# JuliaQuantumControl/GRAPE.jl

Hardware: AMD Instinct MI355X
Metric: GRAPE gradient evals/sec (N=64, 1000 steps, 128 traj) (higher is better)
Workload: dtype f64

## Files before the change

### grape.jl_amd/api.py

```python
from __future__ import annotations

import ctypes as C
import os
import subprocess
import sys

import numpy as np

_HERE = os.path.dirname(os.path.abspath(__file__))
_CSRC = os.path.join(_HERE, "csrc")
_LIBNAME = "libgrape_hip.so"

J_T_SM, J_T_SS, J_T_RE = 0, 1, 2
GRAD_GRADGEN, GRAD_TAYLOR = 0, 1
PROP_EXP, PROP_SERIES = 0, 1
ABI_VERSION = 7

STATUS = {0: "GRAPE_OK", -1: "GRAPE_ERR_INVALID", -2: "GRAPE_ERR_HIP", -3: "GRAPE_ERR_CHI_NORM",
          -4: "GRAPE_ERR_SINGULAR", -5: "GRAPE_ERR_TAYLOR", -6: "GRAPE_ERR_NO_CONTROLS", -7: "GRAPE_ERR_AGAIN",
          -8: "GRAPE_ERR_HOST"}

EXPORTS = ["grape_create", "grape_destroy", "grape_eval", "grape_forward", "grape_backward",
           "grape_forward_device", "grape_backward_device", "grape_check", "grape_get_propagator",
           "grape_get_tau_grads", "grape_get_storage", "grape_get_timings", "grape_reset_timings", "grape_get_work", "grape_get_cert_table",
           "grape_last_error", "grape_abi_version", "grape_set_fused_sweeps", "grape_get_sums", "grape_backward_xi",
           "grape_get_final_states", "grape_backward_chi",
           "grape_get_time_gradient", "grape_set_tlist", "grape_eval_batch", "grape_get_batch_info", "grape_create_open",
           "grape_hvp", "grape_get_hvp_info", "grape_open_time_gradient", "grape_open_hvp", "grape_get_open_hvp_info",
           "grape_open_eval_batch", "grape_get_open_batch_info", "grape_open_set_running_cost", "grape_open_backward_xi",
           "grape_hvp_forward", "grape_hvp_backward", "grape_hvp_backward_chi",
           "grape_open_hvp_forward", "grape_open_hvp_backward", "grape_open_hvp_backward_chi"]


class GrapeHipError(RuntimeError):
    def __init__(self, code, msg):
        super().__init__(f"{STATUS.get(code, code)}: {msg}")
        self.code = code


class _Problem(C.Structure):
    _fields_ = [("abi_version", C.c_int32), ("N", C.c_int32), ("L", C.c_int32), ("K", C.c_int32),
                ("K_total", C.c_int32), ("N_T", C.c_int32), ("functional", C.c_int32),
                ("gradient_method", C.c_int32), ("hc_per_traj", C.c_int32), ("device", C.c_int32),
                ("tlist", C.c_void_p), ("H0", C.c_void_p), ("Hc", C.c_void_p), ("shape", C.c_void_p),
                ("psi0", C.c_void_p), ("target", C.c_void_p), ("weights", C.c_void_p),
                ("chi_min_norm", C.c_double), ("taylor_max_order", C.c_int32),
                ("taylor_tolerance", C.c_double),
                ("Dpen", C.c_void_p), ("dpen_per_traj", C.c_int32), ("lambda_b", C.c_double),
                ("prop_method", C.c_int32), ("prop_tolerance", C.c_double),
                ("ndev", C.c_int32), ("devices", C.c_void_p), ("taylor_no_check", C.c_int32)]


class _Lindblad(C.Structure):
    _fields_ = [("J", C.c_int32), ("cops_per_traj", C.c_int32), ("cops", C.c_void_p)]


def library_path() -> str:
    return os.path.join(_CSRC, _LIBNAME)


def build_asm(verbose: bool = False, workdir: str | None = None) -> str:
    asm_dir = os.path.join(_CSRC, "asm")
    work = workdir or asm_dir
    kernels = (("gen_t16.py", "expm_t16_asm"), ("gen_t16p.py", "expm_t16p_asm"), ("gen_t16p.py", "expm_t16p4_asm"), ("gen_t18g.py", "expm_t18g_asm"), ("gen_t18gp.py", "expm_t18gp_asm"), ("gen_d3.py", "deriv3_asm"), ("gen_d3s.py", "deriv3s_asm"), ("gen_d3s.py", "deriv3g_asm"),
               ("gen_lg.py", "lg_gemm_asm"), ("gen_d4.py", "deriv4_asm_128"), ("gen_d4.py", "deriv4_asm_256"))
    co_path, emb_s, emb_o = os.path.join(work, "grape_asm.co"), os.path.join(work, "asm_embed.S"), os.path.join(work, "asm_embed.o")
    llvm = "/opt/rocm/lib/llvm/bin"
    cmds, objs = [], []
    for gen_py, name in kernels:
        s_path, o_path = os.path.join(work, name + ".s"), os.path.join(work, name + ".o")
        gen = subprocess.run([sys.executable, os.path.join(asm_dir, gen_py), s_path], capture_output=True, text=True)
        if verbose or gen.returncode:
            print(gen.stdout, gen.stderr)
        if gen.returncode:
            raise RuntimeError(gen_py + " failed")
        cmds.append([os.path.join(llvm, "clang"), "-x", "assembler", "-target", "amdgcn-amd-amdhsa", "-mcpu=gfx950", "-c", s_path, "-o", o_path])
        objs.append(o_path)
    cmds.append([os.path.join(llvm, "ld.lld"), "-shared"] + objs + ["-o", co_path])
    with open(emb_s, "w") as f:
        f.write('\t.section .rodata\n\t.globl grape_asm_co_start\n\t.globl grape_asm_co_end\n\t.p2align 12\n'
                'grape_asm_co_start:\n\t.incbin "grape_asm.co"\ngrape_asm_co_end:\n\t.byte 0\n'
                '\t.section .note.GNU-stack,"",@progbits\n')
    cmds.append(["gcc", "-c", "-fPIC", "asm_embed.S", "-o", "asm_embed.o"])
    for c in cmds:
        res = subprocess.run(c, capture_output=True, text=True, cwd=work)
        if verbose or res.returncode:
            print(" ".join(c), res.stdout, res.stderr)
        if res.returncode:
            raise RuntimeError("assembling the gfx950 kernels failed")
    return emb_o


def _sources():
    srcs = [os.path.join(_CSRC, f) for f in ("grape_hip.hip", "grape_t18.hip", "grape_kernels.hip.h", "grape_large.hip.h",
                                             "grape_series.hip.h", "grape_cheby.hip.h", "grape_t18.hip.h", "grape_t18_coeffs.h",
                                             "grape_deriv3.hip.h", "grape_timegrad.hip.h", "grape_batch.hip.h", "grape_lindblad.hip.h", "grape_lindblad_tg.hip.h", "grape_hvp.hip.h", "grape_hvp_split.hip.h", "grape_lindblad_hvp.hip.h", "grape_lindblad_hvp_split.hip.h", "grape_lindblad_batch.hip.h", "grape_lindblad_rc.hip.h", "grape_devmem.h", "grape_cert.hip.h", os.path.join("asm", "gen_t16.py"), os.path.join("asm", "gen_t16p.py"), os.path.join("asm", "gen_t18g.py"), os.path.join("asm", "gen_t18gp.py"), os.path.join("asm", "gen_d3.py"), os.path.join("asm", "gen_d3s.py"), os.path.join("asm", "gen_lg.py"), os.path.join("asm", "gen_d4.py"), os.path.join("asm", "gcn.py"))]
    return srcs, os.path.join(_HERE, "..", "include", "grape_hip.h")


def _up_to_date(out: str) -> bool:
    srcs, hdr = _sources()
    return os.path.exists(out) and all(os.path.getmtime(out) >= os.path.getmtime(s) for s in srcs + [hdr])


def build_library(force: bool = False, verbose: bool = False, extra_flags=(), out: str | None = None) -> str:
    import fcntl
    import shutil
    import tempfile
    out = out or library_path()
    if not force and _up_to_date(out):
        return out
    srcs, _ = _sources()
    with open(os.path.join(_CSRC, ".build.lock"), "w") as lockf:
        fcntl.flock(lockf, fcntl.LOCK_EX)
        if not force and _up_to_date(out):
            return out
        work = tempfile.mkdtemp(prefix="_build_", dir=_CSRC)
        procs = []
        try:
            base = ["hipcc", "--offload-arch=gfx950", "-O3", "-std=c++17", "-fPIC", "-Wno-unused-value"] + list(extra_flags)
            objs = [os.path.join(work, "grape_hip.o"), os.path.join(work, "grape_t18.o")]
            cmds = [base + ["-cuid=grapehip0", "-c", srcs[0], "-o", objs[0]],
                    base + ["-cuid=grapehip1", "-mllvm", "-amdgpu-mfma-vgpr-form", "-c", srcs[1], "-o", objs[1]]]
            procs = [subprocess.Popen(c, stdout=subprocess.PIPE, stderr=subprocess.STDOUT, text=True) for c in cmds]
            objs.append(build_asm(verbose, workdir=work))
            outs = [p.communicate()[0] for p in procs]
            if verbose or any(p.returncode for p in procs):
                print("\n".join(outs))
            if any(p.returncode for p in procs):
                raise RuntimeError("hipcc failed building " + out)
            tmp_so = os.path.join(work, _LIBNAME)
            res = subprocess.run(["hipcc", "--offload-arch=gfx950", "-shared", "-fPIC"] + objs + ["-o", tmp_so], capture_output=True, text=True)
            if verbose or res.returncode:
                print(res.stdout, res.stderr)
            if res.returncode:
                raise RuntimeError("hipcc failed linking " + out)
            asm_dir = os.path.join(_CSRC, "asm")
            for f in os.listdir(work):
                if f.endswith(".s") or f.endswith(".co"):
                    os.replace(os.path.join(work, f), os.path.join(asm_dir, f))
            os.replace(tmp_so, out)
        finally:
            for p in procs:
                if p.poll() is None:
                    p.kill()
                    p.communicate()
            shutil.rmtree(work, ignore_errors=True)
    return out


_lib = None


def load_library():
    global _lib
    if _lib is not None:
        return _lib
    path = library_path()
    if not os.path.exists(path):
        raise GrapeHipError(-2, f"{path} not built; run __graft_entry__.build() (no CPU fallback exists)")
    try:
        import torch
    except ImportError:
        pass
    lib = C.CDLL(path)
    vp, dp, ip = C.c_void_p, C.POINTER(C.c_double), C.c_int
    lib.grape_create.argtypes = [C.POINTER(vp), C.POINTER(_Problem)]
    lib.grape_create_open.argtypes = [C.POINTER(vp), C.POINTER(_Problem), C.POINTER(_Lindblad)]
    lib.grape_destroy.argtypes = [vp]
    lib.grape_destroy.restype = None
    lib.grape_eval.argtypes = [vp, vp, dp, vp, vp, vp]
    lib.grape_forward.argtypes = [vp, vp, vp]
    lib.grape_backward.argtypes = [vp, vp, vp]
    lib.grape_forward_device.argtypes = [vp, vp, vp, vp]
    lib.grape_backward_device.argtypes = [vp, vp, vp, vp]
    lib.grape_check.argtypes = [vp, vp]
    lib.grape_get_propagator.argtypes = [vp, ip, ip, vp]
    lib.grape_get_tau_grads.argtypes = [vp, vp]
    lib.grape_get_storage.argtypes = [vp, ip, vp]
    lib.grape_get_timings.argtypes = [vp, vp, ip]
    lib.grape_get_work.argtypes = [vp, vp, ip]
    lib.grape_get_cert_table.argtypes = [vp, vp, vp, vp]
    lib.grape_reset_timings.argtypes = [vp]
    lib.grape_set_fused_sweeps.argtypes = [vp, ip]
    lib.grape_get_sums.argtypes = [vp, vp]
    lib.grape_get_final_states.argtypes = [vp, vp]
    lib.grape_backward_chi.argtypes = [vp, vp, vp]
    lib.grape_backward_xi.argtypes = [vp, vp, vp, vp, C.c_double, vp]
    lib.grape_get_time_gradient.argtypes = [vp, vp]
    lib.grape_open_time_gradient.argtypes = [vp, vp]
    lib.grape_set_tlist.argtypes = [vp, vp]
    lib.grape_eval_batch.argtypes = [vp, ip, vp, vp, vp, vp]
    lib.grape_get_batch_info.argtypes = [vp, vp, ip]
    lib.grape_hvp.argtypes = [vp, ip, vp, vp]
    lib.grape_get_hvp_info.argtypes = [vp, vp, ip]
    lib.grape_hvp_forward.argtypes = [vp, ip, vp, vp, vp, vp]
    lib.grape_hvp_backward.argtypes = [vp, ip, vp, vp, vp]
    lib.grape_hvp_backward_chi.argtypes = [vp, ip, vp, vp, vp]
    lib.grape_open_hvp.argtypes = [vp, ip, vp, vp]
    lib.grape_get_open_hvp_info.argtypes = [vp, vp, ip]
    lib.grape_open_hvp_forward.argtypes = [vp, ip, vp, vp, vp, vp]
    lib.grape_open_hvp_backward.argtypes = [vp, ip, vp, vp, vp]
    lib.grape_open_hvp_backward_chi.argtypes = [vp, ip, vp, vp, vp]
    lib.grape_open_eval_batch.argtypes = [vp, ip, vp, vp, vp, vp]
    lib.grape_get_open_batch_info.argtypes = [vp, vp, ip]
    lib.grape_open_set_running_cost.argtypes = [vp, vp, ip, C.c_double]
    lib.grape_open_backward_xi.argtypes = [vp, vp, vp, vp, C.c_double, vp]
    lib.grape_last_error.argtypes = [vp]
    lib.grape_last_error.restype = C.c_char_p
    lib.grape_abi_version.restype = ip
    _lib = lib
    return lib


def _c128(a, shape=None):
    a = np.ascontiguousarray(a, dtype=np.complex128)
    if shape is not None:
        assert a.shape == tuple(shape), (a.shape, shape)
    return a


class GrapeHip:

    def __init__(self, H0, Hc, tlist, psi0, target, weights=None, functional=J_T_SM,
                 gradient_method=GRAD_GRADGEN, shape=None, K_total=None, device=0,
                 chi_min_norm=0.0, taylor_max_order=0, taylor_tolerance=0.0, D=None, lambda_b=0.0,
                 prop_method=PROP_EXP, prop_tolerance=0.0, devices=None, taylor_check_convergence=True):
        self._lib = load_library()
        H0 = np.asarray(H0)
        if H0.ndim != 3 or H0.shape[1] != H0.shape[2]:
            raise ValueError(f"H0 must be [K, N, N], got {H0.shape}")
        K, N = H0.shape[0], H0.shape[1]
        Hc = np.asarray(Hc)
        per_traj = Hc.ndim == 4
        if Hc.ndim not in (3, 4) or Hc.shape[-2:] != (N, N) or (per_traj and Hc.shape[0] != K):
            raise ValueError(f"Hc must be [L, N, N] or [K, L, N, N] with N = {N}, K = {K}, got {Hc.shape}")
        L = Hc.shape[1] if per_traj else Hc.shape[0]
        tlist = np.ascontiguousarray(tlist, dtype=np.float64)
        if tlist.ndim != 1 or len(tlist) < 2:
            raise ValueError("tlist must hold at least two time points")
        N_T = len(tlist) - 1
        if weights is not None and np.shape(weights) != (K,):
            raise ValueError(f"weights must be [K] = [{K}], got {np.shape(weights)}")
        if D is not None and np.shape(D) not in ((N, N), (K, N, N)):
            raise ValueError(f"D must be [N, N] or [K, N, N] with N = {N}, K = {K}, got {np.shape(D)}")
        self.N, self.L, self.K, self.N_T = N, L, K, N_T
        self.K_total = K if K_total is None else int(K_total)
        self.functional = functional
        self._H0 = _c128(np.swapaxes(H0, -1, -2), (K, N, N))
        self._Hc = _c128(np.swapaxes(Hc, -1, -2))
        self._psi0 = _c128(psi0, (K, N))
        self._target = None if target is None else _c128(target, (K, N))
        self._tlist = tlist
        self._weights = None if weights is None else np.ascontiguousarray(weights, dtype=np.float64)
        self._shape = None if shape is None else np.ascontiguousarray(shape, dtype=np.float64).reshape(L, N_T)
        p = _Problem()
        p.abi_version = ABI_VERSION
        p.N, p.L, p.K, p.K_total, p.N_T = N, L, K, self.K_total, N_T
        p.functional, p.gradient_method, p.hc_per_traj, p.device = functional, gradient_method, int(per_traj), device
        p.tlist = self._tlist.ctypes.data
        p.H0 = self._H0.ctypes.data
        p.Hc = self._Hc.ctypes.data
        p.shape = None if self._shape is None else self._shape.ctypes.data
        p.psi0 = self._psi0.ctypes.data
        p.target = None if self._target is None else self._target.ctypes.data
# ... 147 lines not shown

    def hvp_forward(self, V, final_states=False):
        v, nv = self._hvp_dirs(V)
        dtau = np.empty((nv, self.K), dtype=np.complex128)
        dsums = np.empty(nv, dtype=np.complex128)
        dpsi = np.empty((nv, self.K, self.N), dtype=np.complex128) if final_states else None
        self._chk(self._lib.grape_hvp_forward(self._h, nv, v.ctypes.data, dtau.ctypes.data, dsums.ctypes.data,
                                              dpsi.ctypes.data if final_states else None))
        if v.ndim == 1:
            dtau, dsums, dpsi = dtau[0], dsums[0], (dpsi[0] if final_states else None)
        return (dtau, dsums, dpsi) if final_states else (dtau, dsums)

    def hvp_backward(self, f_total, df_total):
        one = np.ndim(df_total) == 0
        df = np.ascontiguousarray(df_total, dtype=np.complex128)
        if np.ndim(df_total) > 1 or df.size == 0:
            raise ValueError(f"df_total must be a complex scalar or [nv] with nv >= 1, got {np.shape(df_total)}")
        nv = df.size
        out = np.empty((nv, self.L * self.N_T))
        f = np.array([complex(f_total).real, complex(f_total).imag], dtype=np.float64)
        self._chk(self._lib.grape_hvp_backward(self._h, nv, f.ctypes.data, df.ctypes.data, out.ctypes.data))
        return out[0] if one else out

    def hvp_backward_chi(self, chi, dchi):
        chi = np.ascontiguousarray(chi, dtype=np.complex128)
        d = np.ascontiguousarray(dchi, dtype=np.complex128)
        if chi.shape != (self.K, self.N):
            raise ValueError(f"chi must be [K, N] = [{self.K}, {self.N}], got {chi.shape}")
        if d.ndim not in (2, 3) or d.shape[-2:] != (self.K, self.N) or d.size == 0:
            raise ValueError(f"dchi must be [K, N] = [{self.K}, {self.N}] or [nv, {self.K}, {self.N}] with nv >= 1, got {d.shape}")
        nv = 1 if d.ndim == 2 else d.shape[0]
        out = np.empty((nv, self.L * self.N_T))
        self._chk(self._lib.grape_hvp_backward_chi(self._h, nv, chi.ctypes.data, d.ctypes.data, out.ctypes.data))
        return out[0] if d.ndim == 2 else out

    def set_tlist(self, tlist):
        t = np.ascontiguousarray(tlist, dtype=np.float64)
        if t.shape != (self.N_T + 1,):
            raise ValueError(f"tlist must have N_T + 1 = {self.N_T + 1} points, got {t.shape}")
        self._chk(self._lib.grape_set_tlist(self._h, t.ctypes.data))
        self._tlist = t

    def forward_device(self, d_pulsevals_ptr, d_out_ptr, stream=0):
        self._chk(self._lib.grape_forward_device(self._h, d_pulsevals_ptr, d_out_ptr, stream))

    def backward_device(self, d_f_ptr, d_G_ptr, stream=0):
        self._chk(self._lib.grape_backward_device(self._h, d_f_ptr, d_G_ptr, stream))

    def set_fused_sweeps(self, on=True):
        return bool(self._lib.grape_set_fused_sweeps(self._h, int(bool(on))))

    def check(self, stream=0):
        self._chk(self._lib.grape_check(self._h, stream))

    def propagator(self, k, n):
        out = np.empty((self.N, self.N), dtype=np.complex128)
        self._chk(self._lib.grape_get_propagator(self._h, k, n, out.ctypes.data))
        return out.T.copy()

    def tau_grads(self):
        out = np.empty((self.K, self.L, self.N_T), dtype=np.complex128)
        self._chk(self._lib.grape_get_tau_grads(self._h, out.ctypes.data))
        return out

    def storage(self, which=0):
        out = np.empty((self.K, self.N_T + 1, self.N), dtype=np.complex128)
        self._chk(self._lib.grape_get_storage(self._h, which, out.ctypes.data))
        return out

    def timings(self):
        ms = np.full(8, -1.0)
        self._lib.grape_get_timings(self._h, ms.ctypes.data, 8)
        out = dict(zip(["expm", "forward", "backward", "deriv", "reduce", "total"], ms[:6].tolist()))
        if ms[6] >= 0.0:
            out["host_enqueue"] = float(ms[6])
        if ms[7] >= 0.0:
            out["gradient_allreduce_us"] = float(ms[7]) * 1e3
        return out

    def reset_timings(self):
        self._chk(self._lib.grape_reset_timings(self._h))

    def work(self):
        w = np.zeros(20)
        self._lib.grape_get_work(self._h, w.ctypes.data, 20)
        return dict(cells=w[0], squarings=w[1], flop_expm=w[2], flop_deriv=w[3], deriv_orders=w[4],
                    pivoted_cells=w[5], expm_cells=w[6], series_terms=w[7], series_steps=w[8],
                    t18_mfma_flop=w[9], t18_squarings=w[10], t18_cells=w[11], matrix_free_fallback=w[12], t16_cells=w[13],
                    asm_kernel=w[14], asm_deriv_kernel=w[15], asm_blocked_products=w[16],
                    walk_steps=w[17], scan_block=w[18], t16_certified=w[19])

    def cert_table(self):
        dims = np.zeros(3, np.int32)
        self._chk(self._lib.grape_get_cert_table(self._h, dims.ctypes.data, None, None))
        KC, n8, n6 = (int(x) for x in dims)
        coef, exps = np.zeros((KC, n8 + n6)), np.zeros(n8 + n6, np.int32)
        if n8 + n6:
            self._chk(self._lib.grape_get_cert_table(self._h, dims.ctypes.data, coef.ctypes.data, exps.ctypes.data))
        ex = np.stack([(exps >> (4 * l)) & 15 for l in range(self.L)], axis=1) if n8 + n6 else np.zeros((0, self.L), np.int32)
        return coef[:, :n8], coef[:, n8:], ex


def liouvillian(H, cops=()):
    H = np.asarray(H, dtype=np.complex128)
    d = H.shape[0]
    if H.shape != (d, d):
        raise ValueError(f"H must be [d, d], got {H.shape}")
    eye = np.eye(d)
    heff = H.copy()
    for A in cops:
        A = np.asarray(A, dtype=np.complex128)
        heff = heff - 0.5j * (A.conj().T @ A)
    out = np.kron(eye, heff) - np.kron(heff.conj(), eye)
    for A in cops:
        A = np.asarray(A, dtype=np.complex128)
        out = out + 1j * np.kron(A.conj(), A)
    return out


class GrapeHipOpen(GrapeHip):

    def __init__(self, H0, Hc, cops, tlist, rho0, target, weights=None, functional=J_T_SM, shape=None, K_total=None,
                 device=0, chi_min_norm=0.0, prop_tolerance=0.0):
        self._lib = load_library()
        H0 = np.asarray(H0)
        if H0.ndim != 3 or H0.shape[1] != H0.shape[2]:
            raise ValueError(f"H0 must be [K, d, d], got {H0.shape}")
        K, N = H0.shape[0], H0.shape[1]
        Hc = np.asarray(Hc)
        per_traj = Hc.ndim == 4
        if Hc.ndim not in (3, 4) or Hc.shape[-2:] != (N, N) or (per_traj and Hc.shape[0] != K):
            raise ValueError(f"Hc must be [L, d, d] or [K, L, d, d] with d = {N}, K = {K}, got {Hc.shape}")
        L = Hc.shape[1] if per_traj else Hc.shape[0]
        tlist = np.ascontiguousarray(tlist, dtype=np.float64)
        if tlist.ndim != 1 or len(tlist) < 2:
            raise ValueError("tlist must hold at least two time points")
        N_T = len(tlist) - 1
        if weights is not None and np.shape(weights) != (K,):
            raise ValueError(f"weights must be [K] = [{K}], got {np.shape(weights)}")
        cops = None if cops is None or np.size(cops) == 0 else np.asarray(cops)
        cops_per_traj = cops is not None and cops.ndim == 4
        if cops is not None and (cops.ndim not in (3, 4) or cops.shape[-2:] != (N, N) or (cops_per_traj and cops.shape[0] != K)):
            raise ValueError(f"cops must be [J, d, d] or [K, J, d, d] with d = {N}, K = {K}, got {cops.shape}")
        self.N, self.L, self.K, self.N_T = N, L, K, N_T
        self.J = 0 if cops is None else cops.shape[-3]
        self.K_total = K if K_total is None else int(K_total)
        self.functional = functional
        self.prop_method = PROP_EXP
        self.lambda_b = 0.0
        self._H0 = _c128(np.swapaxes(H0, -1, -2), (K, N, N))
        self._Hc = _c128(np.swapaxes(Hc, -1, -2))
        self._cops = None if cops is None else _c128(np.swapaxes(cops, -1, -2))
        self._psi0 = _c128(np.swapaxes(np.asarray(rho0), -1, -2), (K, N, N))
        self._target = None if target is None else _c128(np.swapaxes(np.asarray(target), -1, -2), (K, N, N))
        self._tlist = tlist
        self._weights = None if weights is None else np.ascontiguousarray(weights, dtype=np.float64)
        self._shape = None if shape is None else np.ascontiguousarray(shape, dtype=np.float64).reshape(L, N_T)
        p = _Problem()
        p.abi_version = ABI_VERSION
        p.N, p.L, p.K, p.K_total, p.N_T = N, L, K, self.K_total, N_T
        p.functional, p.gradient_method, p.hc_per_traj, p.device = functional, GRAD_GRADGEN, int(per_traj), device
        p.tlist = self._tlist.ctypes.data
        p.H0 = self._H0.ctypes.data
        p.Hc = self._Hc.ctypes.data
        p.shape = None if self._shape is None else self._shape.ctypes.data
        p.psi0 = self._psi0.ctypes.data
        p.target = None if self._target is None else self._target.ctypes.data
        p.weights = None if self._weights is None else self._weights.ctypes.data
        p.chi_min_norm = chi_min_norm
        p.prop_method, p.prop_tolerance = PROP_EXP, float(prop_tolerance)
        d = _Lindblad()
        d.J, d.cops_per_traj = self.J, int(cops_per_traj)
        d.cops = None if self._cops is None else self._cops.ctypes.data
        self._h = C.c_void_p()
        rc = self._lib.grape_create_open(C.byref(self._h), C.byref(p), C.byref(d))
        if rc:
            msg = self._lib.grape_last_error(None).decode()
            self._h = None
            raise GrapeHipError(rc, msg)

    def eval(self, pulsevals, gradient=True, want_psiT=False):
        x = np.ascontiguousarray(pulsevals, dtype=np.float64)
        assert x.size == self.L * self.N_T
# ... 143 lines not shown
```

### grape.jl_amd/csrc/asm/gen_d3.py

```python
import os
import struct
import sys

sys.path.insert(0, os.path.dirname(os.path.abspath(__file__)))
from gcn import Prog, V, A, S, VCC, EXEC, Neg, kernel_text

NT = 4
NP = 64
LDT = 17
TILE_B = 16 * LDT * 8
NTILE = NT * (NT + 1) // 2
MAT_B = NTILE * 2 * TILE_B
KERNARG = 160
VPLANE_B = NP * 16 * 16
ECON_MIN = 16
PAIRS_OFF = 32768
ECON_OFF = 32768
ECON_TAB_B = 512


def tile_index(ti, tj):
    assert ti <= tj
    return ti * NT - ti * (ti - 1) // 2 + (tj - ti)


def dbits(x):
    b = struct.unpack("<Q", struct.pack("<d", x))[0]
    return b & 0xFFFFFFFF, b >> 32


class GenD3:
    def __init__(self, name="deriv3_asm", LMAX=2, opts=None):
        assert 1 <= LMAX <= 2
        self.p = Prog(name)
        self.p.soft_vm_flush = True
        self.LMAX = LMAX
        self.opts = dict(opts or {})
        self.lds_bytes = (1 + LMAX) * MAT_B
        self.s_H0, self.s_Hc, self.s_eps, self.s_shape, self.s_dts = S(4, 2), S(6, 2), S(8, 2), S(10, 2), S(12, 2)
        self.s_fw, self.s_bw, self.s_rho = S(14, 2), S(16, 2), S(18, 2)
        self.s_tg, self.s_park, self.s_flags, self.s_stats = S(20, 2), S(22, 2), S(24, 2), S(26, 2)
        self.s_bflag, self.s_inv = S(28, 2), S(30, 2)
        self.s_K, self.s_L, self.s_NT, self.s_hcpt, self.s_wpt, self.s_bpk, self.s_mcap, self.s_maxm = (S(32 + i) for i in range(8))
        self.s_tol2, self.s_deep, self.s_nblk = S(40, 2), S(42), S(43)
        self.s_wave, self.s_slot, self.s_k, self.s_part, self.s_bq, self.s_n0 = (S(44 + i) for i in range(6))
        self.s_m, self.s_M, self.s_conv, self.s_kl = S(50), S(51), S(52), S(53)
        self.s_valid = S(54, 2)
        self.s_fwb, self.s_bwb, self.s_pw = S(56, 2), S(58, 2), S(60, 2)
        self.s_a, self.s_b = S(62, 2), S(64, 2)
        self.s_invm = S(66, 2)
        self.s_t = [S(68 + i) for i in range(8)]
        self.s_pb = [S(76 + 2 * t, 2) for t in range(4)]
        self.s_save = S(84, 2)
        self.s_rhov = S(86, 2)
        self.s_lo16 = S(88, 2)
        self.s_capb, self.s_econ = S(90), S(91)
        self.s_sig = S(92, 2)
        self.v_tid, self.v_lane = V(0), V(1)
        self.v_BD = [V(2 + 2 * op) for op in range(3)]
        self.v_BM = [V(3 + 2 * op) for op in range(3)]
        self.v_fwoff, self.v_bwoff, self.v_poff, self.v_tgoff, self.v_nc8, self.v_zero = V(8), V(9), V(10), V(11), V(12), V(13)
        self.v_dt = V(14, 2)
        self.v_e = [V(16, 2), V(18, 2)]
        self.v_sfac, self.v_nn = V(20, 2), V(22, 2)
        self.v_dr = [V(24, 2), V(28, 2)]
        self.v_di = [V(26, 2), V(30, 2)]
        self.f_re = [V(32 + 2 * rt, 2) for rt in range(4)]
        self.f_im = [V(40 + 2 * rt, 2) for rt in range(4)]
        self.f_as = [V(48 + 2 * rt, 2) for rt in range(4)]
        self.P = [[V(56 + 8 * (4 * j + rt), 8) for rt in range(4)] for j in range(3)]
        self.SUM = [[V(152 + 8 * (4 * j + rt), 8) for rt in range(4)] for j in range(2)]
        self.TMP = [V(216 + 8 * i, 8) for i in range(5)]
        self.VEC = [[A(8 * (4 * j + t), 8) for t in range(4)] for j in range(3)]
        self.CHI = [[A(96 + 8 * (4 * j + t), 8) for t in range(4)] for j in range(2)]
        self.ULAND = A(160, 64)
        self.SHK = [A(224, 2), A(226, 2)]

    def smov64(self, dst, x):
        lo, hi = dbits(x)
        self.p.salu("s_mov_b32", dst.sub(0), lo)
        self.p.salu("s_mov_b32", dst.sub(1), hi)

    def udiv(self, q, r, num, den, tag):
        p = self.p
        i, t = self.s_t[6], self.s_t[7]
        p.salu("s_mov_b32", q, 0)
        p.salu("s_mov_b32", r, 0)
        p.salu("s_mov_b32", i, 31)
        p.label(f"L_div_{tag}")
        p.salu("s_lshl_b32", r, r, 1)
        p.salu("s_lshr_b32", t, num, i)
        p.salu("s_and_b32", t, t, 1)
        p.salu("s_or_b32", r, r, t)
        p.s_cmp("s_cmp_ge_u32", r, den)
        p.s_branch("s_cbranch_scc0", f"L_div_skip_{tag}")
        p.salu("s_sub_u32", r, r, den)
        p.salu("s_lshl_b32", t, 1, i)
        p.salu("s_or_b32", q, q, t)
# ... 581 lines not shown
```

### grape.jl_amd/csrc/grape_cert.hip.h

```cpp
#pragma once

#include <hip/hip_runtime.h>

#include <cstdint>
#include <map>
#include <vector>

#define GRAPE_CERT_LMAX 4

struct CertMonomials {
    std::vector<uint32_t> key;
    std::map<uint32_t, int> index;
    CertMonomials(int M, int d) {
        gen(M, d, 0, 0u);
        for (size_t i = 0; i < key.size(); ++i) index[key[i]] = (int)i;
    }
    int size() const { return (int)key.size(); }

private:
    void gen(int M, int left, int a, uint32_t k) {
        if (a == M - 1) { key.push_back(k | ((uint32_t)left << (4 * a))); return; }
        for (int e = left; e >= 0; --e) gen(M, left - e, a + 1, k | ((uint32_t)e << (4 * a)));
    }
};

struct CertJobs {
    std::vector<int> row, pair;
    void from(const std::vector<std::vector<int>> &lists) {
        row.assign(1, 0);
        pair.clear();
        for (const auto &l : lists) {
            pair.insert(pair.end(), l.begin(), l.end());
            row.push_back((int)pair.size() / 2);
        }
    }
};

struct CertPlan {
    int M, n2, n3, n4, n6, n8, nmat;
    CertJobs mm2, mm34, tr;
    std::vector<int> exps;
    explicit CertPlan(int L) {
        M = L + 1;
        const CertMonomials m2(M, 2), m3(M, 3), m4(M, 4), m6(M, 6), m8(M, 8);
        n2 = m2.size(); n3 = m3.size(); n4 = m4.size(); n6 = m6.size(); n8 = m8.size();
        const int o2 = M, o3 = o2 + n2, o4 = o3 + n3;
        nmat = o4 + n4;
        auto var = [&](int a) { return (uint32_t)1 << (4 * a); };
        std::vector<std::vector<int>> l2(n2), l34(n3 + n4), lt(n8 + n6);
        for (int a = 0; a < M; ++a)
            for (int b = 0; b < M; ++b) { auto &l = l2[m2.index.at(var(a) + var(b))]; l.push_back(a); l.push_back(b); }
        for (int i = 0; i < n2; ++i)
            for (int c = 0; c < M; ++c) { auto &l = l34[m3.index.at(m2.key[i] + var(c))]; l.push_back(o2 + i); l.push_back(c); }
        for (int i = 0; i < n2; ++i)
            for (int j = 0; j < n2; ++j) { auto &l = l34[n3 + m4.index.at(m2.key[i] + m2.key[j])]; l.push_back(o2 + i); l.push_back(o2 + j); }
        for (int i = 0; i < n4; ++i)
            for (int j = 0; j < n4; ++j) { auto &l = lt[m8.index.at(m4.key[i] + m4.key[j])]; l.push_back(o4 + i); l.push_back(o4 + j); }
        for (int i = 0; i < n3; ++i)
            for (int j = 0; j < n3; ++j) { auto &l = lt[n8 + m6.index.at(m3.key[i] + m3.key[j])]; l.push_back(o3 + i); l.push_back(o3 + j); }
        mm2.from(l2); mm34.from(l34); tr.from(lt);
        for (int i = 0; i < n8; ++i) exps.push_back((int)(m8.key[i] >> 4));
        for (int i = 0; i < n6; ++i) exps.push_back((int)(m6.key[i] >> 4));
    }
};

__global__ void __launch_bounds__(256) cert_load_kernel(const double *H0f, const double *Hcf, const int *rep, int kc0, int hc_per_traj, int L,
                                                        int N, int NP, int nmat, double2 *scratch) {
    const int a = blockIdx.x, c = blockIdx.y, kc = kc0 + c, k = rep ? rep[kc] : kc;
    const size_t pp = (size_t)NP * NP;
    const double *src = a == 0 ? H0f + (size_t)k * 2 * pp : Hcf + ((size_t)(hc_per_traj ? k : 0) * L + (a - 1)) * 2 * pp;
    double2 *dst = scratch + ((size_t)c * nmat + a) * N * N;
    for (int e = threadIdx.x; e < N * N; e += 256) {
        const int i = e / N, j = e - i * N;
        dst[e] = make_double2(src[(size_t)i * NP + j], src[pp + (size_t)i * NP + j]);
    }
}

__global__ void __launch_bounds__(256) cert_mm_kernel(double2 *scratch, int nmat, int N, int dst0, const int *row, const int *pair) {
    double2 *base = scratch + (size_t)blockIdx.y * nmat * N * N;
    double2 *dst = base + (size_t)(dst0 + blockIdx.x) * N * N;
    const int p0 = row[blockIdx.x], p1 = row[blockIdx.x + 1];
    for (int e = threadIdx.x; e < N * N; e += 256) {
        const int i = e / N, j = e - i * N;
        double sr = 0., si = 0.;
        for (int q = p0; q < p1; ++q) {
            const double2 *A = base + (size_t)pair[2 * q] * N * N + (size_t)i * N, *B = base + (size_t)pair[2 * q + 1] * N * N + j;
            double tr = 0., ti = 0.;
            for (int k = 0; k < N; ++k) {
                const double2 x = A[k], y = B[(size_t)k * N];
                tr += x.x * y.x - x.y * y.y;
                ti += x.x * y.y + x.y * y.x;
            }
            sr += tr; si += ti;
        }
        dst[e] = make_double2(sr, si);
    }
}

__global__ void __launch_bounds__(256) cert_trace_kernel(const double2 *scratch, int nmat, int N, const int *row, const int *pair, int nt,
                                                         double *table) {
    __shared__ double red[256];
    const double2 *base = scratch + (size_t)blockIdx.y * nmat * N * N;
    const int p0 = row[blockIdx.x], p1 = row[blockIdx.x + 1];
    double sum = 0.;
    for (int q = p0; q < p1; ++q) {
        const double2 *A = base + (size_t)pair[2 * q] * N * N, *B = base + (size_t)pair[2 * q + 1] * N * N;
        double t = 0.;
        for (int e = threadIdx.x; e < N * N; e += 256) {
            const int i = e / N, j = e - i * N;
            const double2 x = A[e], y = B[(size_t)j * N + i];
            t += x.x * y.x - x.y * y.y;
        }
        sum += t;
    }
    red[threadIdx.x] = sum;
    __syncthreads();
    for (int off = 128; off >= 1; off >>= 1) {
        if ((int)threadIdx.x < off) red[threadIdx.x] += red[threadIdx.x + off];
        __syncthreads();
    }
    if (threadIdx.x == 0) table[(size_t)blockIdx.y * nt + blockIdx.x] = red[0];
}
```

### grape.jl_amd/csrc/grape_deriv3.hip.h

```cpp
#pragma once
#include "grape_t18.hip.h"

struct Deriv3Args {
    Deriv2Args d;
    const double *H0f, *Hcf;
    int wpt;
    int skip_if_flagged;
};

template <int NT>
struct D3Lds {
    static constexpr int LDT = 17, TILE = 16 * LDT;
    static constexpr int NTILE = NT * (NT + 1) / 2, MAT = NTILE * 2 * TILE;
    static constexpr int tile(int ti, int tj) { return ti * NT - ti * (ti - 1) / 2 + (tj - ti); }
};

template <int NT>
struct D3Vec {
    d4 re[NT], im[NT];
};
template <int NT>
__device__ __forceinline__ void d3_finish(D3Vec<NT> &) {}
#define MFMA64_NEGA(a, b, c) __builtin_amdgcn_mfma_f64_16x16x4f64((a), (b), (c), 0, 0, 1)

// ... 90 lines not shown
#pragma unroll
                    for (int tj = 0; tj < NT; ++tj) {
                        const bool full = H0G && m == 0;
                        if (tj < ti && !full) continue;
                        const size_t o = (size_t)(16 * ti + row) * NP + 16 * tj + col;
                        const int q_ = full ? ti * NT + tj : LY::tile(ti, tj);
                        double *dst = d3sm + (m == 0 ? (size_t)0 : (size_t)H0SZ + (size_t)(m - 1) * LY::MAT) + (size_t)q_ * 2 * LY::TILE
                                      + row * LY::LDT + col;
                        dst[0] = src[o];
                        dst[LY::TILE] = src[pp + o];
                    }
            }
            __syncthreads();
            k_loaded = k;
        }
        for (int bq = part * 4 + wave; bq < a.batches_per_k; bq += 4 * g.wpt) {
            const int batch = k * a.batches_per_k + bq;
            const int n0 = bq * 16, n = n0 + c;
            const bool valid = n < a.N_T;
            const int nc = valid ? n : a.N_T - 1;
            const double dt = a.dts[nc];
            double e[LMAX], sh[LMAX];
#pragma unroll
            for (int l = 0; l < LMAX; ++l) {
                sh[l] = (l < L && a.shape) ? a.shape[(size_t)l * a.N_T + nc] : 1.0;
                e[l] = l < L ? a.eps[(size_t)l * a.N_T + nc] * sh[l] : 0.;
            }
            auto apply = [&](const D3Vec<NT> &v, Strip<NT> &sum, auto each, auto adj) __attribute__((always_inline)) {
                if constexpr (!H0G) d3_product<NT, D3_HERM>(sum, d3sm, v, lane);
                else if constexpr (decltype(adj)::value) d3_product<NT, D3_FULL_ADJ>(sum, d3sm, v, lane);
                else d3_product<NT, D3_FULL>(sum, d3sm, v, lane);
#pragma unroll
                for (int l = 0; l < LMAX; ++l) {
                    if (l < L) {
                        Strip<NT> q;
                        d3_product<NT, D3_HERM>(q, d3sm + (size_t)H0SZ + (size_t)l * LY::MAT, v, lane);
                        each(l, q);
#pragma unroll
                        for (int t = 0; t < NT; ++t) { sum.re[t] += e[l] * q.re[t]; sum.im[t] += e[l] * q.im[t]; }
                    }
                }
            };
            D3Vec<NT> v;
#pragma unroll
            for (int t = 0; t < NT; ++t)
#pragma unroll
                for (int r = 0; r < 4; ++r) {
                    const int row = 16 * t + 4 * r + rg;
                    const double2 p = a.fw[((size_t)k * (a.N_T + 1) + nc) * NP + row];
                    v.re[t][r] = valid ? p.x : 0.; v.im[t][r] = valid ? p.y : 0.;
                    const size_t o = (size_t)row * 16 + c;
                    park[o] = v.re[t][r]; park[vplane + o] = v.im[t][r];
                }
            d3_finish<NT>(v);
            int M = 0, converged = 0;
            const int deg = (a.batch_econ && a.batch_flag && a.econ_pairs) ? a.batch_flag[a.nbatch_total + batch] : 0;
            const int capb = (deg && deg - 1 <= mcap) ? deg - 1 : mcap;
            const double *pairs = nullptr;
            for (int m = 1; m <= capb; ++m) {
                Strip<NT> sum;
                apply(v, sum, [](int, const Strip<NT> &) {}, std::false_type());
                const double sfac = dt / (double)m;
                double nn = 0.;
#pragma unroll
                for (int t = 0; t < NT; ++t)
#pragma unroll
                    for (int r = 0; r < 4; ++r) {
                        const double ur = sfac * sum.im[t][r], ui = -sfac * sum.re[t][r];
                        v.re[t][r] = ur; v.im[t][r] = ui;
                        if (m < a.maxm) {
                            const size_t o = (size_t)m * 2 * vplane + (size_t)(16 * t + 4 * r + rg) * 16 + c;
                            park[o] = ur; park[vplane + o] = ui;
                        }
                        nn += ur * ur + ui * ui;
                    }
                d3_finish<NT>(v);
                nn += __shfl_xor(nn, 16, 64);
                nn += __shfl_xor(nn, 32, 64);
                M = m;
                if (m >= 2 && __all(nn < a.tol * a.tol)) { converged = 1; break; }
            }
            if (!converged && capb != mcap) {
                M = deg; converged = 1;
                pairs = a.econ_pairs + (size_t)(deg - 16) * 64;
            }
            Strip<NT> chi;
#pragma unroll
            for (int t = 0; t < NT; ++t)
#pragma unroll
                for (int r = 0; r < 4; ++r) {
                    const int row = 16 * t + 4 * r + rg;
                    const double2 x = a.bw[((size_t)k * (a.N_T + 1) + nc + 1) * NP + row];
                    chi.re[t][r] = valid ? x.x : 0.; chi.im[t][r] = valid ? x.y : 0.;
                    v.re[t][r] = chi.re[t][r]; v.im[t][r] = chi.im[t][r];
                }
            d3_finish<NT>(v);
            double dr[LMAX], di[LMAX];
#pragma unroll
            for (int l = 0; l < LMAX; ++l) { dr[l] = 0.; di[l] = 0.; }
            for (int aa = M - 1; aa >= 0; --aa) {
                const double inv = pairs ? pairs[2 * aa] : 1.0 / (double)(aa + 1), sfac = dt * (pairs ? pairs[2 * aa + 1] : inv);
                Strip<NT> u;
#pragma unroll
                for (int t = 0; t < NT; ++t)
#pragma unroll
                    for (int r = 0; r < 4; ++r) {
                        const size_t o = (size_t)aa * 2 * vplane + (size_t)(16 * t + 4 * r + rg) * 16 + c;
                        u.re[t][r] = park[o]; u.im[t][r] = park[vplane + o];
                    }
                Strip<NT> sum;
                apply(v, sum, [&](int l, const Strip<NT> &q) {
                    double sr = 0., si = 0.;
#pragma unroll
                    for (int t = 0; t < NT; ++t)
#pragma unroll
                        for (int r = 0; r < 4; ++r) {
                            sr += q.re[t][r] * u.re[t][r] + q.im[t][r] * u.im[t][r];
                            si += q.re[t][r] * u.im[t][r] - q.im[t][r] * u.re[t][r];
                        }
#pragma unroll
                    for (int ll = 0; ll < LMAX; ++ll)
                        if (ll == l) { dr[ll] += inv * sr; di[ll] += inv * si; }
                }, std::true_type());
                if (aa > 0) {
#pragma unroll
                    for (int t = 0; t < NT; ++t) {
                        v.re[t] = chi.re[t] - sfac * sum.im[t];
                        v.im[t] = chi.im[t] + sfac * sum.re[t];
                    }
                    d3_finish<NT>(v);
                }
            }
            const double rho = a.rho[k];
#pragma unroll
            for (int l = 0; l < LMAX; ++l) {
                if (l < L) {
                    double Dr = dr[l], Di = di[l];
                    Dr += __shfl_xor(Dr, 16, 64); Di += __shfl_xor(Di, 16, 64);
                    Dr += __shfl_xor(Dr, 32, 64); Di += __shfl_xor(Di, 32, 64);
                    if (lane < 16 && valid) {
                        const double f = rho * dt * sh[l];
                        a.tg[((size_t)k * L + l) * a.N_T + n] = make_double2(f * Di, -f * Dr);
                    }
                }
            }
            if (lane == 0) {
                const bool redone = a.batch_flag && a.batch_flag[batch];
                if (!converged && !redone) {
                    if (a.deep_redo && a.max_order > mcap) atomicAdd(&a.flags[7], 1);
                    else atomicOr(&a.flags[0], 4);
                }
                if (!redone) stat_add(a.stats, 8, (unsigned long long)M * (unsigned long long)min(16, a.N_T - n0));
            }
        }
    }
}
```

### grape.jl_amd/csrc/grape_econ_coeffs.h

```cpp
#pragma once
#define ECON_NSETS 4
#define ECON_MAXDEG 21
static const int ECON_DEG[4] = {16, 17, 19, 21};
static const double ECON_THETAS[4] = {1.36, 1.6, 2.0, 2.72};
static const double ECON_TABS[4][21][2] = {
    {
        {0.99999999999999980529, 0.0},
        {0.49999999999999995125, 0.5000000000000000486},
        {0.33333333333332434652, 0.33333333333332437902},
        {0.24999999999999620304, 0.25000000000000294314},
        {0.19999999999926497087, 0.19999999999926800844},
        {0.16666666666628327988, 0.16666666666689580415},
        {0.14285714278897023749, 0.14285714278929885474},
        {0.12499999995893169073, 0.12500000001858273294},
        {0.11111110479818800082, 0.11111110483469316255},
        {0.099999995732971707361, 0.10000000141460258699},
        {0.09090855395893132458, 0.090908557838025207959},
        {0.083332932906864668469, 0.083333425111719705549},
        {0.076884663733727549698, 0.07688503317535548076},
        {0.071397325340398044236, 0.071432996940482527776},
        {0.064640984384933717337, 0.064669273650506011373},
        {0.06071810592472735844, 0.062620855279837302966},
    },
    {
        {0.99999999999999999455, 0.0},
        {0.4999999999999993495, 0.49999999999999935223},
        {0.33333333333333310332, 0.33333333333333353698},
        {0.24999999999996339023, 0.24999999999996356274},
        {0.19999999999998274025, 0.20000000000001202807},
        {0.16666666666399540022, 0.16666666666400978334},
        {0.14285714285565865098, 0.14285714285794830793},
        {0.12499999979320799999, 0.12499999979450668039},
        {0.11111111098113255448, 0.11111111116494766568},
        {0.099999984471020328113, 0.099999984588001011055},
        {0.090909080095443414331, 0.090909094212698174517},
        {0.08333227990005947407, 0.083332289812445550663},
        {0.076922274865354993361, 0.07692324726745345143},
        {0.071369128617731144553, 0.071369872773579570035},
        {0.066617645519177640728, 0.066673130855455625664},
        {0.060046505756126821541, 0.060090691475870164317},
        {0.056647927484758038627, 0.058962556159000548588},
    },
    {
        {0.99999999999999999921, 0.0},
        {0.49999999999999992552, 0.49999999999999992591},
        {0.33333333333333330714, 0.33333333333333335679},
        {0.24999999999999664644, 0.24999999999999666609},
        {0.19999999999999844313, 0.20000000000000112597},
        {0.16666666666646977996, 0.16666666666647107735},
        {0.14285714285703602551, 0.14285714285720478555},
        {0.12499999998758439536, 0.12499999998767787304},
        {0.11111111110354300887, 0.11111111111457910189},
        {0.099999999224287985445, 0.099999999231099277407},
        {0.090909090388332223524, 0.090909091093524965459},
        {0.08333328800342905667, 0.083333288480790928176},
        {0.076923043819425117041, 0.076923085662418433957},
        {0.071426233987298557027, 0.071426264725411121612},
        {0.066664825888945511032, 0.066667007511954072934},
        {0.062401392779846247146, 0.062403115833826611183},
        {0.058740346168331276547, 0.058833168170990150001},
        {0.052549019651987751242, 0.052623435248405465345},
        {0.04992966106659680109, 0.052786333172829262077},
    },
    {
        {0.99999999999999999857, 0.0},
        {0.49999999999999991112, 0.49999999999999991184},
        {0.33333333333333330218, 0.33333333333333336144},
        {0.24999999999999735495, 0.24999999999999737832},
        {0.19999999999999878645, 0.20000000000000090249},
        {0.16666666666656360018, 0.16666666666656461147},
        {0.14285714285708797303, 0.14285714285717631573},
        {0.12499999999564817792, 0.12499999999569620152},
        {0.11111111110852316905, 0.11111111111239145534},
        {0.099999999815243407927, 0.099999999817572555781},
        {0.090909090788705288148, 0.090909090956665826485},
        {0.083333325825673231936, 0.083333325936026708004},
        {0.076923071625269883499, 0.076923078555417816465},
        {0.071428292264000648122, 0.071428297183374011482},
        {0.066666455064462201818, 0.066666715618252914584},
        {0.06249097939752106286, 0.062491177746585624593},
        {0.058816230400073814299, 0.058824720550794186756},
        {0.055319711558037046927, 0.055326576656644222471},
        {0.052428888318170015129, 0.052652407896601588093},
        {0.04557403849702946584, 0.045750228205306646811},
        {0.043596611933927011585, 0.047830533974697739686},
    },
};
```

### grape.jl_amd/csrc/grape_hip.hip

```cpp
#include "../../include/grape_hip.h"
#include "grape_kernels.hip.h"
#include "grape_t18_coeffs.h"
#include "grape_econ_coeffs.h"
#include "grape_large.hip.h"
#include "grape_series.hip.h"
#include "grape_cheby.hip.h"
#include "grape_timegrad.hip.h"
#include "grape_lindblad.hip.h"
#include "grape_lindblad_tg.hip.h"
#include "grape_hvp.hip.h"
#include "grape_hvp_split.hip.h"
#include "grape_lindblad_hvp.hip.h"
#include "grape_lindblad_hvp_split.hip.h"
#include "grape_lindblad_batch.hip.h"
#include "grape_lindblad_rc.hip.h"
#include "grape_devmem.h"
#include "grape_cert.hip.h"

#include <rccl/rccl.h>
#include <dlfcn.h>
#include <mutex>

#include <algorithm>
#include <chrono>
// ... 6 lines not shown
#include <string>
#include <thread>
#include <vector>

namespace {

thread_local std::string g_create_error;

int barrier_fail(std::string *err, const char *what) noexcept {
    try {
        *err = std::string("host-side C++ exception caught at the C boundary: ") + what;
    } catch (...) {
    }
    return -8;
}
#define GRAPE_BARRIER(errptr)                                                                                   \
    catch (const std::bad_alloc &) { return barrier_fail((errptr), "std::bad_alloc (out of host memory)"); }    \
    catch (const std::exception &e) { return barrier_fail((errptr), e.what()); }                                \
    catch (...) { return barrier_fail((errptr), "unknown exception"); }

void test_throw_point(const char *where) {
    const char *hk = getenv("GRAPE_TEST_HOOKS");
    if (!(hk && atoi(hk) == 1)) return;
    const char *t = getenv("GRAPE_TEST_THROW"), *at = getenv("GRAPE_TEST_THROW_AT");
    if (!t || strcmp(at ? at : "early", where)) return;
    if (!strcmp(t, "bad_alloc")) throw std::bad_alloc();
    throw std::runtime_error(t);
}

constexpr int kRing = 64;
constexpr int kPhases = 6;
struct Phase { hipEvent_t e0, e1; bool used; };

}

struct OpenCtx;

struct grape_handle {
    grape_problem p{};
    int N = 0, NP = 0, NT = 0, L = 0, K = 0, K_total = 0, N_T = 0;
    int device = 0;
    hipStream_t stream = nullptr;
    double *d_H0f = nullptr, *d_Hcf = nullptr, *d_H0t = nullptr, *d_Hct = nullptr;
    double *d_H0p = nullptr, *d_Hcp = nullptr, *d_vecs = nullptr;
    double *d_H0q = nullptr, *d_Hcq = nullptr, *d_park2 = nullptr;
    double *d_H0q3 = nullptr, *d_Hcq3 = nullptr, *d_H0p3 = nullptr, *d_Hcp3 = nullptr;
    int deriv4_blocks = 0;
    double *d_park3 = nullptr;
    int deriv3_blocks = 0, deriv3_wpt = 0;
    bool deriv3_h0g = false;
    bool deriv3_general = false;
    int deriv2 = 0, deriv2_maxm = 0;
    bool deriv_stream = false;
    bool deriv_stream_never = false;
    int deriv_blocks = 0;
    bool large = false;
    int chunk = 0;
    double *d_lg[9] = {nullptr, nullptr, nullptr, nullptr, nullptr, nullptr, nullptr, nullptr, nullptr};
    double *d_dinv = nullptr;
    int *d_scell = nullptr;
    double *d_colpart = nullptr;
    bool lg_form2 = false;
    double *d_normpart = nullptr;
    double *d_dts = nullptr, *d_shape = nullptr, *d_weights = nullptr;
    double2 *d_psi0 = nullptr, *d_target = nullptr;
    double *d_eps = nullptr;
    double2 *d_U = nullptr, *d_fw = nullptr, *d_bw = nullptr, *d_tg = nullptr;
    double *d_ret = nullptr;
    double *d_out = nullptr;
    double *d_f = nullptr, *d_G = nullptr, *d_rho = nullptr;
    int *d_flags = nullptr;
    int *d_cellflag = nullptr;
    int KC = 0;
    bool herm = false;
    bool herm_ctrl = false;
    bool t18 = false;
    bool t18_small = true;
    bool t16 = true;
    double *d_gram = nullptr;
    int *d_celllist = nullptr;
    double *d_cert = nullptr;
    int *d_cert_exp = nullptr;
    int cert_n8 = 0, cert_n6 = 0;
    bool asm16 = false;
    bool asm16p = false;
    double *d_dte = nullptr;
    bool asm18gp = false;
    bool asm18g = false;
    int *d_wgtab = nullptr, *d_prog = nullptr, *d_splan = nullptr;
    double2 *d_xinit = nullptr;
    int asm_blocks = 0;
    int last_walk_fuse = 0;
    bool asm_sq = true;
    int asm_walk = 0;
    bool foreign_stream = false;
    bool credit_pending = false;
    std::vector<double> bal;
    std::vector<double> bal_stage_chi, bal_stage_xi;
    double *d_Sf = nullptr;
    bool expm_persist = true;
    int expm_lds_pad_kb = 0;
    bool test_hooks = false;
    bool lg_asm = true;
    bool deriv3_asm = true;
    bool taylor_check = true;
    bool no_target = false;
    std::vector<int> cls;
    int *d_cls = nullptr, *d_rep = nullptr;
    int coop_S = 0;
    int *d_xcc_sw = nullptr;
    int coop_rpw = 0, coop_nw = 0;
    double2 *d_Dt = nullptr, *d_xi = nullptr;
    double *d_wq = nullptr, *d_gb = nullptr;
    bool have_gb = false;
    const double2 *xi_user = nullptr;
    double lambda_user = 0.0;
    unsigned long long *d_stats = nullptr;
    double *h_pin = nullptr;
    DeviceBufs mem;
    size_t h_pin_doubles = 0;
    Phase ph[kRing][kPhases]{};
    long n_fwd = 0, n_bwd = 0;
    std::string err;
    bool have_forward = false, in_eval = false;
    double chi_min_norm = 1e-100, taylor_tol = 1e-16;
    int taylor_max_order = 100;
    bool fuse = false;
    bool fuse_on = true;
    bool want_bw = true;
    bool bw_done = false;
    bool bw_unit = false;
    bool z_valid = false;
    double *d_inv_tnorm = nullptr, *d_ones = nullptr;
    double2 *d_z = nullptr;
    bool scan16 = false;
    int scan_Bk = 0, scan_NB = 0;
    double2 *d_scanF = nullptr, *d_scan_fw = nullptr, *d_scan_bw = nullptr;
    int num_cus = 256;
    bool series = false;
    bool u_fallback = false;
    double *d_rb = nullptr;
    double series_tol = 1e-17, series_theta = 3.0;
    double *d_n1 = nullptr;
    double2 *d_gpark = nullptr;
    int *d_morder = nullptr;
    int maxp = 0;
    int *d_batchflag = nullptr;
    bool deriv_econ = false;
    const double *d_econ_pairs = nullptr;
    int *d_celldeg = nullptr;
    double sub_theta = 0.0;
    int sq_plan = 2;
    double2 *d_xch = nullptr;
    int *d_xcc = nullptr;
    int cheby_S = 0, cheby_round = 0, cheby_pair = 0;
    double2 *d_chi_in = nullptr;
    std::vector<grape_handle *> shards;
    std::vector<int> shard_lo;
    std::vector<int> shard_dev;
    bool use_rccl = false;
    void *comm_set = nullptr;
    std::vector<double *> d_red;
    bool rccl_fwd_checked = false, rccl_bwd_checked = false;
    hipEvent_t ar0 = nullptr, ar1 = nullptr;
    double allreduce_ms = 0.0;
    long allreduce_calls = 0;
// ... 2614 lines not shown
        CCHK(h->mem.alloc(&h->d_wgtab, tab.size()));
        CCHK(h->mem.alloc(&h->d_splan, (size_t)ncell));
        CCHK(hipMemset(h->d_splan, 0, (size_t)ncell * sizeof(int)));
        CCHK(hipMemcpy(h->d_wgtab, tab.data(), tab.size() * sizeof(int), hipMemcpyHostToDevice));
        const char *envw = getenv("GRAPE_EXPM_WALK"), *envq = getenv("GRAPE_EXPM_SQ");
        h->asm_sq = !(envq && atoi(envq) == 0);
        h->asm_walk = h->KC == K ? (envw ? atoi(envw) & 3 : 3) : 0;
        if (h->scan16) h->asm_walk = 0;
        if (h->asm_walk) {
            std::vector<double> xi((size_t)2 * K * 64 * 2, 0.0);
            for (int k = 0; k < K; ++k) {
                double n2 = 0.0;
                for (int i = 0; i < 2 * N; ++i) n2 += p->target[(size_t)k * 2 * N + i] * p->target[(size_t)k * 2 * N + i];
                const double itn = n2 > 0.0 ? 1.0 / std::sqrt(n2) : 0.0;
                for (int i = 0; i < N; ++i) {
                    xi[2 * ((size_t)k * 64 + i)] = p->psi0[2 * ((size_t)k * N + i)];
                    xi[2 * ((size_t)k * 64 + i) + 1] = p->psi0[2 * ((size_t)k * N + i) + 1];
                    xi[2 * ((size_t)(K + k) * 64 + i)] = p->target[2 * ((size_t)k * N + i)] * itn;
                    xi[2 * ((size_t)(K + k) * 64 + i) + 1] = -p->target[2 * ((size_t)k * N + i) + 1] * itn;
                }
            }
            CCHK(h->mem.alloc(&h->d_xinit, (size_t)2 * K * 64));
            CCHK(hipMemcpy(h->d_xinit, xi.data(), xi.size() * 8, hipMemcpyHostToDevice));
            CCHK(h->mem.alloc(&h->d_prog, (size_t)2 * K));
            CCHK(hipMemset(h->d_prog, 0, (size_t)2 * K * sizeof(int)));
        }
    }
    if (h->t16 && h->t18 && h->herm && !h->large && !h->series && (h->NT >= 3 || (h->NT == 2 && h->t18_small))) {
        CCHK(h->mem.alloc(&h->d_celllist, (size_t)K * N_T));
        const int M = L + 1, KCn = h->KC;
        const int GS = M * M + M;
        std::vector<double> gram((size_t)KCn * GS);
        std::vector<int> repk(KCn, -1);
        auto shape_factor = [&](const double *op, double fro2) {
            if (!(fro2 > 0.0)) return 1.0;
            std::vector<double> a2((size_t)2 * N * N), a4((size_t)2 * N * N);
            auto square = [&](const double *a, std::vector<double> &c) {
                std::fill(c.begin(), c.end(), 0.0);
                for (int j = 0; j < N; ++j)
                    for (int k = 0; k < N; ++k) {
                        const double br = a[2 * ((size_t)j * N + k)], bi = a[2 * ((size_t)j * N + k) + 1];
                        const double *ak = a + 2 * (size_t)k * N;
                        double *cj = &c[2 * (size_t)j * N];
                        for (int i = 0; i < N; ++i) {
                            cj[2 * i] += ak[2 * i] * br - ak[2 * i + 1] * bi;
                            cj[2 * i + 1] += ak[2 * i] * bi + ak[2 * i + 1] * br;
                        }
                    }
            };
            square(op, a2);
            square(a2.data(), a4);
            double m8 = 0.0;
            for (double x : a4) m8 += x * x;
            const double s8 = std::pow(m8, 0.125), semi = std::pow(3.5, 0.125) * 2.0 * std::sqrt(fro2 / (double)N);
            const double kap = s8 / semi;
            return std::isfinite(kap) && kap > 0.0 ? kap : 1.0;
        };
        std::vector<double> kap_shared((size_t)L, -1.0);
        for (int k = K - 1; k >= 0; --k) repk[h->cls.empty() ? k : h->cls[k]] = k;
        const size_t nn2 = (size_t)2 * N * N;
        for (int kc = 0; kc < KCn; ++kc) {
            const int k = repk[kc] < 0 ? kc : repk[kc];
            auto op = [&](int a) { return a == 0 ? p->H0 + (size_t)k * nn2 : p->Hc + ((size_t)(p->hc_per_traj ? k : 0) * L + (a - 1)) * nn2; };
            for (int a = 0; a < M; ++a)
                for (int b = a; b < M; ++b) {
                    const double *x = op(a), *y = op(b);
                    double sum = 0.;
                    for (size_t i = 0; i < nn2; ++i) sum += x[i] * y[i];
                    gram[(size_t)kc * GS + (size_t)a * M + b] = gram[(size_t)kc * GS + (size_t)b * M + a] = sum;
                }
        }
        if (!p->hc_per_traj)
            for (int l = 0; l < L; ++l) kap_shared[l] = shape_factor(p->Hc + (size_t)l * nn2, gram[(size_t)(1 + l) * M + (1 + l)]);
        parallel_for(KCn, [&](int kc) {
            const int k = repk[kc] < 0 ? kc : repk[kc];
            for (int a = 0; a < M; ++a) {
                const double fro2 = gram[(size_t)kc * GS + (size_t)a * M + a];
                const double *o = a == 0 ? p->H0 + (size_t)k * nn2 : p->Hc + ((size_t)(p->hc_per_traj ? k : 0) * L + (a - 1)) * nn2;
                gram[(size_t)kc * GS + (size_t)M * M + a] = (a > 0 && !p->hc_per_traj) ? kap_shared[a - 1] : shape_factor(o, fro2);
            }
        });
        CCHK(h->mem.alloc(&h->d_gram, gram.size()));
        CCHK(hipMemcpy(h->d_gram, gram.data(), gram.size() * 8, hipMemcpyHostToDevice));
        const char *envc = getenv("GRAPE_EXPM_CERT");
        if (h->asm16 && L >= 1 && L <= GRAPE_CERT_LMAX && !(envc && atoi(envc) == 0)) {
            const CertPlan pl(L);
            const int nt = pl.n8 + pl.n6;
            h->cert_n8 = pl.n8; h->cert_n6 = pl.n6;
            CCHK(h->mem.alloc(&h->d_cert, (size_t)KCn * nt));
            CCHK(h->mem.alloc(&h->d_cert_exp, (size_t)nt));
            CCHK(hipMemcpy(h->d_cert_exp, pl.exps.data(), (size_t)nt * sizeof(int), hipMemcpyHostToDevice));
            DeviceBufs tmp;
            int *d_job[6] = {nullptr, nullptr, nullptr, nullptr, nullptr, nullptr};
            const std::vector<int> *job[6] = {&pl.mm2.row, &pl.mm2.pair, &pl.mm34.row, &pl.mm34.pair, &pl.tr.row, &pl.tr.pair};
            for (int i = 0; i < 6; ++i) {
                CCHK(tmp.alloc(&d_job[i], job[i]->size()));
                CCHK(hipMemcpy(d_job[i], job[i]->data(), job[i]->size() * sizeof(int), hipMemcpyHostToDevice));
            }
            const size_t per_class = (size_t)pl.nmat * N * N;
            const int chunk = (int)std::max<size_t>(1, std::min<size_t>((size_t)KCn, ((size_t)64 << 20) / (per_class * sizeof(double2))));
            double2 *d_scr = nullptr;
            CCHK(tmp.alloc(&d_scr, per_class * chunk));
            for (int kc0 = 0; kc0 < KCn; kc0 += chunk) {
                const unsigned nc = (unsigned)std::min(chunk, KCn - kc0);
                hipLaunchKernelGGL(cert_load_kernel, dim3((unsigned)pl.M, nc), dim3(256), 0, 0, (const double *)h->d_H0f, (const double *)h->d_Hcf,
                                   (const int *)h->d_rep, kc0, p->hc_per_traj ? 1 : 0, L, N, NP, pl.nmat, d_scr);
                hipLaunchKernelGGL(cert_mm_kernel, dim3((unsigned)pl.n2, nc), dim3(256), 0, 0, d_scr, pl.nmat, N, pl.M, (const int *)d_job[0], (const int *)d_job[1]);
                hipLaunchKernelGGL(cert_mm_kernel, dim3((unsigned)(pl.n3 + pl.n4), nc), dim3(256), 0, 0, d_scr, pl.nmat, N, pl.M + pl.n2, (const int *)d_job[2],
                                   (const int *)d_job[3]);
                hipLaunchKernelGGL(cert_trace_kernel, dim3((unsigned)nt, nc), dim3(256), 0, 0, (const double2 *)d_scr, pl.nmat, N, (const int *)d_job[4],
                                   (const int *)d_job[5], nt, h->d_cert + (size_t)kc0 * nt);
                CCHK(hipGetLastError());
            }
            CCHK(hipDeviceSynchronize());
        }
    }
    if (h->large && h->series) {
        const int per_xcd = std::max(1, h->num_cus / 8), S = h->NP / 16;
        if (per_xcd < S) {
            h->err = "prop_method = GRAPE_PROP_SERIES with N > 64 needs NP / 16 co-resident workgroups per XCD";
            return fail(GRAPE_ERR_INVALID);
        }
        h->cheby_S = S;
        h->cheby_pair = h->fuse && per_xcd >= 2 * S;
        if (!h->cheby_pair) h->fuse = false;
        h->cheby_round = 8 * std::max(1, per_xcd / ((h->cheby_pair ? 2 : 1) * S));
        CCHK(h->mem.alloc(&h->d_xch, (size_t)2 * K * 4 * NP));
        CCHK(h->mem.alloc(&h->d_xcc, (size_t)2 * K * 32));
    }
    if (h->large && !h->series) {
        hipDeviceProp_t prop;
        CCHK(hipGetDeviceProperties(&prop, h->device));
        const int per_xcd = std::max(1, prop.multiProcessorCount / 8), groups = (K + 7) / 8;
        int S = 1;
        while (S * 2 * groups <= per_xcd && h->NP / (S * 2) >= 4) S *= 2;
        const int R = h->NP / S;
        const char *env = getenv("GRAPE_SWEEP_COOP");
        if (S >= 2 && R <= 64 && !(env && atoi(env) == 0)) {
            h->coop_S = S;
            h->coop_nw = R >= 16 ? 16 : R;
            h->coop_rpw = R / h->coop_nw;
            CCHK(h->mem.alloc(&h->d_xcc_sw, (size_t)2 * K * 32));
        }
    }
    CCHK(hipMemset(h->d_flags, 0, 8 * sizeof(int)));
    CCHK(hipMemset(h->d_stats, 0, (size_t)GRAPE_STAT_SHARDS * GRAPE_STAT_SLOTS * sizeof(unsigned long long)));
    CCHK(hipMemset(h->d_fw, 0, (size_t)K * (N_T + 1) * NP * 16));
    CCHK(hipMemset(h->d_bw, 0, (size_t)K * (N_T + 1) * NP * 16));
    CCHK(hipMemset(h->d_tg, 0, (size_t)K * L * N_T * 16));
    h->h_pin_doubles = (size_t)2 * L * N_T + 2 * K + 16;
    if (p->Dpen && p->lambda_b != 0.0) {
        h->have_gb = true;
        const int Kd = p->dpen_per_traj ? K : 1;
        std::vector<double> dt_((size_t)Kd * pp * 2, 0.0);
        for (int kd = 0; kd < Kd; ++kd)
            for (int j = 0; j < N; ++j)
                for (int i = 0; i < N; ++i) {
                    dt_[2 * ((size_t)kd * pp + (size_t)j * NP + i)] = p->Dpen[2 * ((size_t)kd * nn + (size_t)j * N + i)];
                    dt_[2 * ((size_t)kd * pp + (size_t)j * NP + i) + 1] = p->Dpen[2 * ((size_t)kd * nn + (size_t)j * N + i) + 1];
                }
        CCHK(h->mem.alloc(&h->d_Dt, (size_t)Kd * pp));
        CCHK(hipMemcpy(h->d_Dt, dt_.data(), dt_.size() * 8, hipMemcpyHostToDevice));
        std::vector<double> wq(N_T + 1);
        for (int m = 0; m <= N_T; ++m)
            wq[m] = m == 0 ? (p->tlist[1] - p->tlist[0]) / 2.0
                           : (m < N_T ? 0.5 * (p->tlist[m + 1] - p->tlist[m - 1]) : (p->tlist[N_T] - p->tlist[N_T - 1]) / 2.0);
        CCHK(h->mem.alloc(&h->d_wq, (size_t)N_T + 1));
        CCHK(hipMemcpy(h->d_wq, wq.data(), wq.size() * 8, hipMemcpyHostToDevice));
        CCHK(h->mem.alloc(&h->d_xi, (size_t)K * (N_T + 1) * NP));
        CCHK(h->mem.alloc(&h->d_gb, (size_t)K * (N_T + 1)));
    }
    {
        h->batch_ok = !h->large && !h->series && NP == 16 && h->t18 && h->t18_small && p->gradient_method == GRAPE_GRAD_GRADGEN &&
                      !h->have_gb && h->fuse && !h->no_target && h->K == h->K_total && !h->test_hooks && L <= 8;
        if (const char *envb = getenv("GRAPE_BATCH")) h->batch_env = atoi(envb) != 0 ? 1 : 0;
        if (const char *envs = getenv("GRAPE_BATCH_SETS")) h->batch.store.env = std::max(0, atoi(envs));
        if (const char *envh = getenv("GRAPE_HVP_DIRS")) h->hvp.store.env = std::max(0, atoi(envh));
    }
    CCHK(h->mem.alloc_pinned(&h->h_pin, h->h_pin_doubles));
    CCHK(hipDeviceSynchronize());
#undef CCHK
    test_throw_point("late");
    *out = guard.release();
    return GRAPE_OK;
}
GRAPE_BARRIER(&g_create_error)

int grape_forward_device(grape_handle *h, const double *d_pulsevals, double *d_out, void *stream_) try {
    if (h && h->open) return open_refuse(h, "grape_forward_device");
    if (!h || !d_pulsevals || !d_out) return GRAPE_ERR_INVALID;
    if (!h->shards.empty()) { h->err = "device-pointer entry points need a single-device handle (ndev <= 1)"; return GRAPE_ERR_INVALID; }
    hipStream_t s = (hipStream_t)stream_;
    h->foreign_stream = s != h->stream;
    HIPCHK(h, hipSetDevice(h->device));
    (void)hipGetLastError();
    HIPCHK(h, hipMemsetAsync(h->d_flags, 0, 8 * sizeof(int) + (size_t)GRAPE_STAT_SHARDS * GRAPE_STAT_SLOTS * sizeof(unsigned long long), s));
    if (d_pulsevals != h->d_eps)
        HIPCHK(h, hipMemcpyAsync(h->d_eps, d_pulsevals, (size_t)h->L * h->N_T * 8, hipMemcpyDeviceToDevice, s));
    ExpmArgs ea{};
    ea.H0f = h->d_H0f; ea.Hcf = h->d_Hcf; ea.eps = h->d_eps; ea.shape = h->d_shape; ea.dts = h->d_dts;
    ea.U = h->d_U; ea.flags = h->d_flags; ea.stats = h->d_stats; ea.cellflag = h->d_cellflag;
    ea.K = h->KC; ea.rep = h->d_rep; ea.L = h->L; ea.N_T = h->N_T; ea.hc_per_traj = h->p.hc_per_traj;
    ea.n1 = h->d_n1; ea.n1_k = h->K;
#ifdef GRAPE_DIAG
    ea.ablate = getenv("GRAPE_DIAG_ABLATE") ? atoi(getenv("GRAPE_DIAG_ABLATE")) : 0;
    static unsigned long long *d_stamps = nullptr;
    if (getenv("GRAPE_DIAG_STAMPS")) {
        if (!d_stamps) hipMalloc((void **)&d_stamps, (size_t)h->K * h->N_T * 32 * 8);
        hipMemsetAsync(d_stamps, 0, (size_t)h->K * h->N_T * 32 * 8, s);
    }
    ea.stamps = d_stamps;
    hipMemcpyToSymbolAsync(HIP_SYMBOL(g_diag_slot_base), &d_stamps, sizeof(d_stamps), 0, hipMemcpyHostToDevice, s);
    grape_t18_set_stamps(d_stamps, (void *)s);
#endif
    hipError_t e = hipSuccess;
    int walk_fuse = 0;
    if (!h->series) {
        phase_begin(h, 0, s);
        if (h->large) {
            e = h->t18 ? expm_large_t18(h, s) : expm_large(h, s);
        } else {
            const long ncell = (long)ea.K * ea.N_T;
            const int per_cu = h->NT == 1 ? 10 : h->NT == 2 ? 4 : 1;
            const int t18_blocks = 8 * (int)std::max<long>(1, std::min<long>((long)(h->num_cus / 8) * per_cu, (ncell + 7) / 8));
            if (h->t18 && (h->NT >= 3 || h->t18_small)) {
                if (h->d_Sf) {
                    CtrlSumArgs ca{};
                    ca.Hcf = h->d_Hcf; ca.eps = h->d_eps; ca.shape = h->d_shape; ca.Sf = h->d_Sf;
                    ca.L = h->L; ca.N_T = h->N_T; ca.pp2 = 2 * h->NP * h->NP;
                    ca.per_traj = h->p.hc_per_traj ? 1 : 0; ca.rep = h->d_rep;
                    hipLaunchKernelGGL(ctrl_sum_kernel, dim3((unsigned)((ca.per_traj ? h->KC : 1) * h->N_T), std::max(1, ca.pp2 / 2 / 2048)), dim3(256), 0, s, ca);
                    HIPCHK(h, hipGetLastError());
                    ea.Sf = h->d_Sf;
                }
                const bool t16 = h->d_celllist != nullptr;
                ea.cell_list = h->d_celllist; ea.listed = 0;
                if (t16) {
                    T16PlanArgs pa{};
                    pa.gram = h->d_gram; pa.eps = h->d_eps; pa.shape = h->d_shape; pa.dts = h->d_dts; pa.flags = h->d_flags;
                    pa.KC = h->KC; pa.L = h->L; pa.N_T = h->N_T; pa.N = h->N;
                    pa.splan = (h->asm16 && (h->asm_sq || h->d_cert)) ? h->d_splan : nullptr;
                    pa.sq_on = h->asm_sq ? 1 : 0;
                    pa.cert = h->d_cert; pa.cert_exp = h->d_cert_exp; pa.n8 = h->cert_n8; pa.n6 = h->cert_n6;
                    pa.verdict = h->d_cellflag;
                    hipLaunchKernelGGL(t16_plan_kernel, dim3((unsigned)((ncell + 255) / 256)), dim3(256), 0, s, pa);
                    HIPCHK(h, hipGetLastError());
                }
                const int blocks16 = (t16 && h->NT == 3) ? 8 * (int)std::max<long>(1, std::min<long>((long)(h->num_cus / 8) * 2, (ncell + 7) / 8)) : t18_blocks;
                h->credit_pending = false;
                if (h->asm18g) {
                    walk_fuse = h->asm_walk & (1 | ((h->fuse && h->fuse_on && h->want_bw) ? 2 : 0));
                    if (walk_fuse) HIPCHK(h, hipMemsetAsync(h->d_prog, 0, (size_t)2 * h->K * sizeof(int), s));
                    const void *walk[6] = {h->d_wgtab, h->d_xinit, h->d_fw, h->d_bw, h->d_prog, h->d_splan};
                    if (h->asm18gp) {
                        hipLaunchKernelGGL(dte_kernel, dim3((unsigned)((h->N_T + 255) / 256)), dim3(256), 0, s, (const double *)h->d_eps,
                                           (const double *)h->d_shape, (const double *)h->d_dts, h->L, h->N_T, 2, h->d_dte);
                        HIPCHK(h, hipGetLastError());
                    }
                    e = (hipError_t)grape_t18g_asm_launch(&ea, sizeof(ea), h->d_cellflag, (void *)s, h->asm_blocks, walk, walk_fuse, h->K,
                                                          h->asm18gp ? h->d_dte : nullptr);
                    h->credit_pending = !h->asm18gp;
                }
                else if (t16 && h->asm16p) {
                    walk_fuse = h->asm_walk & (1 | ((h->fuse && h->fuse_on && h->want_bw) ? 2 : 0));
                    if (walk_fuse) HIPCHK(h, hipMemsetAsync(h->d_prog, 0, (size_t)2 * h->K * sizeof(int), s));
                    hipLaunchKernelGGL(dte_kernel, dim3((unsigned)((h->N_T + 255) / 256)), dim3(256), 0, s, (const double *)h->d_eps,
                                       (const double *)h->d_shape, (const double *)h->d_dts, h->L, h->N_T, h->L <= 2 ? 2 : 4, h->d_dte);
                    HIPCHK(h, hipGetLastError());
                    const void *walk[6] = {h->d_wgtab, h->d_xinit, h->d_fw, h->d_bw, h->d_prog, h->d_splan};
                    e = (hipError_t)grape_t16p_asm_launch(&ea, sizeof(ea), h->d_cellflag, (void *)s, h->asm_blocks, walk, walk_fuse, h->K, h->d_dte);
                }
                else if (t16 && h->asm16) {
                    walk_fuse = h->asm_walk & (1 | ((h->fuse && h->fuse_on && h->want_bw) ? 2 : 0));
                    if (walk_fuse) HIPCHK(h, hipMemsetAsync(h->d_prog, 0, (size_t)2 * h->K * sizeof(int), s));
                    const void *walk[6] = {h->d_wgtab, h->d_xinit, h->d_fw, h->d_bw, h->d_prog, h->d_splan};
                    e = (hipError_t)grape_t16_asm_launch(&ea, sizeof(ea), h->d_cellflag, (void *)s, h->asm_blocks, walk, walk_fuse, h->K);
                    h->credit_pending = true;
                }
                else
                    e = (hipError_t)grape_t18_launch(h->NT, h->herm ? 1 : 0, t16 ? 1 : 0, &ea, sizeof(ea), (void *)s, blocks16);
                if (t16 && e == hipSuccess) {
                    ea.listed = 1;
                    e = (hipError_t)grape_t18_launch(h->NT, 1, 0, &ea, sizeof(ea), (void *)s, t18_blocks);
                }
            } else
            switch (h->NT) {
                case 1: e = launch_expm<1>(ea, h->herm, s, 0, h->expm_lds_pad_kb); break;
                case 2: e = launch_expm<2>(ea, h->herm, s, 0, h->expm_lds_pad_kb); break;
                case 3: e = launch_expm<3>(ea, h->herm, s, 0, h->expm_lds_pad_kb); break;
                default: {
                    const int nb = 8 * (h->num_cus / 8);
                    const bool persist = h->expm_persist && nb >= 8 && (long)ea.K * ea.N_T >= 4L * nb;
                    e = launch_expm<4>(ea, h->herm, s, persist ? nb : 0, h->expm_lds_pad_kb);
                    break;
                }
            }
        }
        HIPCHK(h, e);
        if (h->deriv_econ) {
            DerivEconArgs ec{};
            ec.verdict = h->d_cellflag; ec.splan = h->d_splan; ec.cls = h->d_cls; ec.flags = h->d_flags;
            ec.cell_deg = h->large ? h->d_celldeg : nullptr;
            ec.deg0 = ECON_DEG[0]; ec.deg1 = ECON_DEG[ECON_NSETS - 1];
            static_assert(ECON_NSETS == 4, "segments 1.36 (verdict), 1.6, 2.0 (blocked path), 2.72 (one planned squaring)");
            ec.K = h->K; ec.KC = h->KC; ec.N_T = h->N_T; ec.batches_per_k = (h->N_T + 15) / 16;
            ec.nbatch_total = h->K * ec.batches_per_k; ec.batch_econ = h->d_batchflag + ec.nbatch_total;
            hipLaunchKernelGGL(deriv_econ_kernel, dim3((unsigned)((ec.nbatch_total + 255) / 256)), dim3(256), 0, s, ec);
            HIPCHK(h, hipGetLastError());
        }
        phase_end(h, 0, s);
    }
#ifdef GRAPE_DIAG
    if (ea.stamps) {
        hipStreamSynchronize(s);
        const size_t nb = (size_t)h->KC * h->N_T;
        std::vector<unsigned long long> st(nb * 32);
        hipMemcpy(st.data(), ea.stamps, nb * 32 * 8, hipMemcpyDeviceToHost);
        auto avg = [&](int i1, int i0) {
            double sum = 0;
            size_t cnt = 0;
            for (size_t b = 0; b < nb; ++b)
                if (st[b * 32 + i1] && st[b * 32 + i0]) { sum += (double)(st[b * 32 + i1] - st[b * 32 + i0]); ++cnt; }
            return cnt ? sum / cnt : 0.0;
        };
        if (h->t18 && h->NT >= 3) {
            const char *tn[] = {"form A (+norm)", "A2 = A A + half exchange", "A3 = A A2", "store A3, norm A2, barrier", "A6 = A3 A3",
                                "A6 exchanges + norms", "scaling, B1 -> X, barrier", "A9 = B1 B5", "+B4, B3+A9 -> X, B2", "p = B2 + (B3+A9) A9",
                                "squarings", "store U", "end barrier"};
            for (int j = 0; j < 13; ++j) fprintf(stderr, "  stamp %-28s %9.0f cycles\n", tn[j], avg(j + 1, j));
            fprintf(stderr, "  stamp %-28s %9.0f cycles\n", "TOTAL per cell", avg(13, 0));
        } else {
        const char *pn[] = {"form A", "norm", "A2", "A4,A6 (+store A2)", "store A6 + combos", "dual", "U=A*T"};
        for (int j = 0; j < 7; ++j) fprintf(stderr, "  stamp %-24s %9.0f cycles\n", pn[j], avg(11 + j, j ? 10 + j : 0));
        fprintf(stderr, "  stamp %-24s %9.0f cycles\n", "P,Q + first inversion", avg(5, 17));
        fprintf(stderr, "  stamp   barrier %6.0f, P/Q stores %6.0f, barrier %6.0f, strip loads + barrier + I_0 %6.0f\n", avg(26, 17), avg(27, 26), avg(28, 27), avg(5, 28));
        fprintf(stderr, "  stamp   strip loads + barrier %6.0f, then wave 0 (I_0) %6.0f, wave 1 (tiles + prefetch) %6.0f, wave 2 (prefetch) %6.0f\n", avg(22, 28), avg(29, 22), avg(30, 22), avg(31, 22));
        for (int j = 0; j < 4; ++j) fprintf(stderr, "  stamp solve step %d             %9.0f cycles\n", j, avg(6 + j, 5 + j));
        for (int j = 0; j < 1; ++j)
            fprintf(stderr, "  stamp   step %d, waves done after %6.0f %6.0f %6.0f %6.0f cycles\n", j, avg(18 + 4 * j, 5 + j),
                    avg(19 + 4 * j, 5 + j), avg(20 + 4 * j, 5 + j), avg(21 + 4 * j, 5 + j));
        fprintf(stderr, "  stamp %-24s %9.0f cycles\n", "squarings + store U", avg(4, 3));
        fprintf(stderr, "  stamp %-24s %9.0f cycles\n", "TOTAL per cell", avg(4, 0));
        }
    }
#endif
    h->last_walk_fuse = walk_fuse;
    h->tg_state = h->want_bw ? 2 : 1;
    h->hvs.came(grape_handle::HvpSplit::EVAL);
    SweepArgs sa{};
    sa.U = h->d_U; sa.cls = h->d_cls; sa.psi0 = h->d_psi0; sa.target = h->d_target; sa.weights = h->d_weights;
    sa.store = h->d_fw; sa.tau = (double2 *)d_out; sa.f = nullptr; sa.rho = h->d_rho; sa.flags = h->d_flags;
    sa.chi_min_norm = h->chi_min_norm;
    sa.K = h->K; sa.K_total = h->K_total; sa.N = h->N; sa.N_T = h->N_T; sa.functional = h->p.functional;
    sa.xcc = h->d_xcc_sw;
    if (walk_fuse & 1) sa.resume = h->d_prog;
    if (h->test_hooks) {
        const char *envd = getenv("GRAPE_TEST_DROP_SIBLING");
        sa.drop_sibling = envd ? atoi(envd) : 0;
    }
    phase_begin(h, 1, s);
    const bool pair = h->fuse && h->fuse_on && h->want_bw;
    h->bw_done = h->bw_unit = pair;
    h->z_valid = false;
    if (pair) {
        SweepArgs sb = sa;
        sb.store = h->d_bw; sb.tau = (double2 *)h->d_out; sb.f = nullptr; sb.unit_chi = 1; sb.inv_tnorm = h->d_inv_tnorm;
        sb.resume = (walk_fuse & 2) ? h->d_prog + h->K : nullptr;
        if (h->series && h->large) {
            e = launch_cheby(h, &sa, &sb, s);
        } else if (h->series) {
            const SeriesArgs rf = series_args(h, sa, false), rb = series_args(h, sb, true);
            const bool sc = 2 * h->K > h->num_cus;
            e = h->NP == 16 ? launch_series_pair<16>(rf, rb, sc, s) : h->NP == 32 ? launch_series_pair<32>(rf, rb, sc, s)
                                                                                 : launch_series_pair<64>(rf, rb, sc, s);
        } else if (h->scan16) {
            e = launch_scan(h, &sa, &sb, true, s);
        } else {
            e = h->NP == 16 ? launch_sweep_pair<16>(sa, sb, s) : h->NP == 32 ? launch_sweep_pair<32>(sa, sb, s)
                : h->NP == 48 ? launch_sweep_pair<48>(sa, sb, s) : launch_sweep_pair<64>(sa, sb, s);
        }
    } else if (h->series && h->large) {
        e = launch_cheby(h, &sa, nullptr, s);
    } else if (h->series) {
        const SeriesArgs ra = series_args(h, sa, false);
        e = h->NP == 16 ? launch_series<16>(ra, false, s) : h->NP == 32 ? launch_series<32>(ra, false, s)
                                                                       : launch_series<64>(ra, false, s);
    } else if (h->scan16) {
// ... 850 lines not shown
        return GRAPE_ERR_INVALID;
    }
    HIPCHK(h, hipSetDevice(h->device));
    HIPCHK(h, hipDeviceSynchronize());
    const size_t pp = (size_t)h->NP * h->NP;
    std::vector<double> tmp(2 * pp);
    HIPCHK(h, hipMemcpy(tmp.data(), h->d_U + ((size_t)h->cls[k] * h->N_T + n) * pp, pp * 16, hipMemcpyDeviceToHost));
    for (int j = 0; j < h->N; ++j)
        for (int i = 0; i < h->N; ++i) {
            const double f = h->bal.empty() ? 1.0 : h->bal[i] / h->bal[j];
            out[2 * ((size_t)j * h->N + i)] = f * tmp[2 * ((size_t)i * h->NP + j)];
            out[2 * ((size_t)j * h->N + i) + 1] = f * tmp[2 * ((size_t)i * h->NP + j) + 1];
        }
    return GRAPE_OK;
}
GRAPE_BARRIER(h ? &h->err : &g_create_error)

int grape_get_timings(grape_handle *h, double *ms, int n) try {
    if (!h || !ms) return GRAPE_ERR_INVALID;
    if (h->open) {
        const OpenCtx *o = h->open;
        const double f = o->n_fwd ? o->ms_fwd / o->n_fwd : -1.0, b = o->n_bwd ? o->ms_bwd / o->n_bwd : -1.0;
        const double v[kPhases] = {0.0, f, b, 0.0, 0.0, f < 0.0 ? -1.0 : f + std::max(b, 0.0)};
        int cnt = 0;
        for (; cnt < kPhases && cnt < n; ++cnt) ms[cnt] = v[cnt];
        return cnt;
    }
    if (!h->shards.empty()) {
        int cnt = 0;
        for (size_t g = 0; g < h->shards.size(); ++g) {
            double cm[kPhases];
            cnt = grape_get_timings(h->shards[g], cm, n < kPhases ? n : kPhases);
            if (cnt < 0) return multi_fail(h, h->shards[g], cnt);
            for (int i = 0; i < cnt; ++i) ms[i] = g == 0 ? cm[i] : std::max(ms[i], cm[i]);
        }
        if (n > kPhases) { ms[kPhases] = h->host_enqueue_calls ? 2.0 * h->host_enqueue_ms / h->host_enqueue_calls : -1.0; cnt = kPhases + 1; }
        if (n > kPhases + 1) { ms[kPhases + 1] = (h->use_rccl && h->allreduce_calls) ? h->allreduce_ms / h->allreduce_calls : -1.0; cnt = kPhases + 2; }
        return cnt;
    }
    HIPCHK(h, hipSetDevice(h->device));
    HIPCHK(h, hipDeviceSynchronize());
    int cnt = 0;
    for (int i = 0; i < kPhases && i < n; ++i, ++cnt) {
        double sum = 0.0;
        int used = 0;
        for (int r = 0; r < kRing; ++r) {
            float t = 0.f;
            Phase &p = h->ph[r][i];
            if (p.used && hipEventElapsedTime(&t, p.e0, p.e1) == hipSuccess) { sum += t; ++used; }
        }
        ms[i] = used ? sum / used : -1.0;
    }
    return cnt;
}
GRAPE_BARRIER(h ? &h->err : &g_create_error)

int grape_reset_timings(grape_handle *h) try {
    if (!h) return GRAPE_ERR_INVALID;
    if (h->open) { h->open->ms_fwd = h->open->ms_bwd = 0.0; h->open->n_fwd = h->open->n_bwd = 0; return GRAPE_OK; }
    if (!h->shards.empty()) {
        for (grape_handle *c : h->shards) {
            const int rc = grape_reset_timings(c);
            if (rc) return multi_fail(h, c, rc);
        }
        h->host_enqueue_ms = 0.0;
        h->allreduce_ms = 0.0; h->allreduce_calls = 0;
        h->host_enqueue_calls = 0;
        return GRAPE_OK;
    }
    HIPCHK(h, hipSetDevice(h->device));
    HIPCHK(h, hipDeviceSynchronize());
    for (auto &ring : h->ph)
        for (auto &p : ring) p.used = false;
    h->n_fwd = h->n_bwd = 0;
    h->n_eval = 0;
    return GRAPE_OK;
}
GRAPE_BARRIER(h ? &h->err : &g_create_error)

int grape_get_work(grape_handle *h, double *out, int n) try {
    if (!h || !out || n < 4) return GRAPE_ERR_INVALID;
    if (h->open) return open_work(h, out, n);
    if (!h->shards.empty()) {
        const int m = n < 20 ? n : 20;
        std::fill(out, out + m, 0.0);
        for (grape_handle *c : h->shards) {
            double cw[20] = {0.};
            const int rc = grape_get_work(c, cw, m);
            if (rc < 0) return multi_fail(h, c, rc);
            for (int i = 0; i < m; ++i) out[i] = (i == 15 || i == 16 || i == 18) ? cw[i] : out[i] + cw[i];
        }
        if (m > 14 && out[14] > 0.0) out[14] = h->shards[0]->asm16p ? 3.0 : h->shards[0]->asm18gp ? 4.0 : h->shards[0]->asm18g ? 2.0 : 1.0;
        return 4;
    }
    HIPCHK(h, hipSetDevice(h->device));
    HIPCHK(h, hipDeviceSynchronize());
    if (h->credit_pending) {
        ExpmArgs ea{};
        ea.H0f = h->d_H0f; ea.Hcf = h->d_Hcf; ea.eps = h->d_eps; ea.shape = h->d_shape; ea.dts = h->d_dts;
        ea.flags = h->d_flags; ea.stats = h->d_stats; ea.Sf = h->d_Sf;
        ea.K = h->KC; ea.rep = h->d_rep; ea.L = h->L; ea.N_T = h->N_T; ea.hc_per_traj = h->p.hc_per_traj;
        ea.n1 = h->d_n1; ea.n1_k = h->K;
        HIPCHK(h, (hipError_t)grape_t16_credit_launch(&ea, sizeof(ea), (void *)h->stream));
        HIPCHK(h, hipStreamSynchronize(h->stream));
        h->credit_pending = false;
    }
    unsigned long long sh[GRAPE_STAT_SHARDS * GRAPE_STAT_SLOTS], st[GRAPE_STAT_SLOTS] = {0};
    HIPCHK(h, hipMemcpy(sh, h->d_stats, sizeof(sh), hipMemcpyDeviceToHost));
    for (int q = 0; q < GRAPE_STAT_SHARDS; ++q)
        for (int i = 0; i < GRAPE_STAT_SLOTS; ++i) st[i] += sh[q * GRAPE_STAT_SLOTS + i];
    const double N3 = (double)h->N * h->N * h->N, N2 = (double)h->N * h->N;
    const double cells = (double)h->K * h->N_T, ecells = (double)h->KC * h->N_T;
    const double gemms = 2.0 * st[3] + 3.0 * st[4] + 4.0 * st[5] + 5.0 * st[6] + 6.0 * st[7];
    out[0] = cells;
    out[1] = (double)st[0];
    out[2] = (gemms + (double)st[0]) * 8.0 * N3 + ecells * (32.0 / 3.0) * N3;
    out[3] = (double)st[8] * (1.0 + 2.0 * h->L) * 8.0 * N2;
    if (n > 4) out[4] = (double)st[8];
    if (n > 5) out[5] = (double)st[9];
    if (n > 6) out[6] = h->series ? 0.0 : ecells;
    if (n > 7) out[7] = (double)st[10];
    if (n > 8) out[8] = (double)st[11];
    if (n > 9) out[9] = (double)st[12] * 2048.0;
    if (n > 10) out[10] = (double)st[13];
    if (n > 11) out[11] = (double)st[14];
    if (n > 12) out[12] = h->u_fallback ? 1.0 : 0.0;
    if (n > 13) out[13] = (double)st[15];
    if (n > 14) out[14] = h->asm16p ? 3.0 : h->asm16 ? 1.0 : h->asm18gp ? 4.0 : h->asm18g ? 2.0 : 0.0;
    if (n > 15) {
        double kind = 0.0;
        if (!h->series && h->d_park3 && h->NT == 4) {
            if (h->deriv3_general) kind = 3.0;
            else if (h->L > 2) kind = 2.0;
            else if (!h->deriv3_h0g && h->deriv3_asm) kind = 1.0;
        } else if (!h->series && h->deriv4_blocks) kind = 4.0;
        out[15] = kind;
    }
    if (n > 16) out[16] = (h->large && !h->series && h->t18 && h->lg_asm) ? 1.0 : 0.0;
    if (n > 17) {
        double carried = 0.0;
        if (h->last_walk_fuse && h->d_prog) {
            std::vector<int> prog((size_t)2 * h->K);
            HIPCHK(h, hipMemcpy(prog.data(), h->d_prog, prog.size() * sizeof(int), hipMemcpyDeviceToHost));
            for (int k = 0; k < h->K; ++k) {
                if (h->last_walk_fuse & 1) carried += prog[(size_t)k];
                if (h->last_walk_fuse & 2) carried += prog[(size_t)h->K + k];
            }
        }
        out[17] = carried;
    }
    if (n > 18) out[18] = h->scan16 ? (double)h->scan_Bk : 0.0;
    if (n > 19) {
        double certified = 0.0;
        if (h->d_cert && h->d_splan && !h->series) {
            const size_t ncell = (size_t)h->KC * h->N_T;
            std::vector<int> plan(ncell);
            int fl[8];
            HIPCHK(h, hipMemcpy(plan.data(), h->d_splan, ncell * sizeof(int), hipMemcpyDeviceToHost));
            HIPCHK(h, hipMemcpy(fl, h->d_flags, sizeof(fl), hipMemcpyDeviceToHost));
            if (!(4L * fl[6] > (long)ncell))
                for (int w : plan) certified += (w & T16_PLAN_CERT) ? 1.0 : 0.0;
        }
        out[19] = certified;
    }
    return 4;
}
GRAPE_BARRIER(h ? &h->err : &g_create_error)

int grape_get_cert_table(grape_handle *h, int *dims, double *coef, int *exps) try {
    if (!h || !dims) return GRAPE_ERR_INVALID;
    if (h->open || !h->shards.empty()) {
        h->err = "grape_get_cert_table: a closed handle on one device";
        return GRAPE_ERR_INVALID;
    }
    const int nt = h->cert_n8 + h->cert_n6;
    dims[0] = h->KC; dims[1] = h->cert_n8; dims[2] = h->cert_n6;
    if (!h->d_cert || !nt) { dims[1] = dims[2] = 0; return GRAPE_OK; }
    HIPCHK(h, hipSetDevice(h->device));
    if (coef) HIPCHK(h, hipMemcpy(coef, h->d_cert, (size_t)h->KC * nt * sizeof(double), hipMemcpyDeviceToHost));
    if (exps) HIPCHK(h, hipMemcpy(exps, h->d_cert_exp, (size_t)nt * sizeof(int), hipMemcpyDeviceToHost));
    return GRAPE_OK;
}
GRAPE_BARRIER(h ? &h->err : &g_create_error)

int grape_get_time_gradient(grape_handle *h, double *dJdt) try {
    if (h && h->open) return open_refuse(h, "grape_get_time_gradient");
    if (!h || !dJdt) return GRAPE_ERR_INVALID;
    const int N_T = h->N_T;
    if (!h->shards.empty()) {
        std::vector<double> part((size_t)N_T);
        for (size_t g = 0; g < h->shards.size(); ++g) {
            const int rc = grape_get_time_gradient(h->shards[g], g == 0 ? dJdt : part.data());
            if (rc) return multi_fail(h, h->shards[g], rc);
            if (g > 0) for (int n = 0; n < N_T; ++n) dJdt[n] += part[n];
        }
        return GRAPE_OK;
    }
    if (h->tg_state != 3) {
        h->err = h->tg_state == 0 ? "grape_get_time_gradient: no complete gradient evaluation on this time grid (none yet, the last "
                                    "one failed, or grape_set_tlist came after it)"
               : h->tg_state == 1 ? "grape_get_time_gradient: the last evaluation had no gradient (grape_eval with G == NULL)"
                                  : "grape_get_time_gradient called between grape_forward and the backward half";
        return GRAPE_ERR_INVALID;
    }
    HIPCHK(h, hipSetDevice(h->device));
    if (h->foreign_stream) HIPCHK(h, hipDeviceSynchronize());
    (void)hipGetLastError();
    if (!h->d_tq) HIPCHK(h, h->mem.alloc(&h->d_tq, (size_t)h->K * N_T));
    if (!h->d_dJdt) HIPCHK(h, h->mem.alloc(&h->d_dJdt, (size_t)N_T));
    TimeGradArgs ta{};
    ta.H0f = h->d_H0f; ta.Hcf = h->d_Hcf; ta.eps = h->d_eps; ta.shape = h->d_shape;
    ta.fw = h->d_fw; ta.bw = h->d_bw; ta.rho = h->d_rho; ta.z = h->tg_unit ? h->d_z : nullptr;
    ta.gb = (h->have_gb && !h->tg_xi_user) ? h->d_gb : nullptr; ta.lambda_q = 0.25 * h->p.lambda_b;
    ta.out = h->d_tq;
    ta.K = h->K; ta.L = h->L; ta.N = h->N; ta.NP = h->NP; ta.N_T = N_T; ta.hc_per_traj = h->p.hc_per_traj;
    const int nct = h->NP <= 64 ? 4 : h->NP <= 128 ? 2 : 1;
    const size_t lds = (size_t)2 * h->NP * 16 * nct * sizeof(double);
    const dim3 grid((unsigned)((N_T + 16 * nct - 1) / (16 * nct)), (unsigned)h->K);
    int dev = 0;
    HIPCHK(h, hipGetDevice(&dev));
    static LdsLimit lim1, lim2, lim4;
    if (nct == 4) {
        HIPCHK(h, lim4.ensure((const void *)time_grad_kernel<4>, dev, lds));
        hipLaunchKernelGGL(time_grad_kernel<4>, grid, dim3(256), lds, h->stream, ta);
    } else if (nct == 2) {
        HIPCHK(h, lim2.ensure((const void *)time_grad_kernel<2>, dev, lds));
        hipLaunchKernelGGL(time_grad_kernel<2>, grid, dim3(256), lds, h->stream, ta);
    } else {
        HIPCHK(h, lim1.ensure((const void *)time_grad_kernel<1>, dev, lds));
        hipLaunchKernelGGL(time_grad_kernel<1>, grid, dim3(256), lds, h->stream, ta);
    }
    HIPCHK(h, hipGetLastError());
    hipLaunchKernelGGL(grad_reduce_kernel, dim3((N_T + 15) / 16), dim3(256), 0, h->stream, h->d_tq, h->K, N_T, h->d_dJdt,
                       (const double2 *)nullptr);
    HIPCHK(h, hipGetLastError());
    HIPCHK(h, hipMemcpyAsync(dJdt, h->d_dJdt, (size_t)N_T * 8, hipMemcpyDeviceToHost, h->stream));
    HIPCHK(h, hipStreamSynchronize(h->stream));
    return GRAPE_OK;
}
GRAPE_BARRIER(h ? &h->err : &g_create_error)

int grape_open_time_gradient(grape_handle *h, double *dJdt) try {
    if (!h) { g_create_error = "grape_open_time_gradient: h == NULL"; return GRAPE_ERR_INVALID; }
    if (!dJdt) { h->err = "grape_open_time_gradient: dJdt == NULL"; return GRAPE_ERR_INVALID; }
    if (!h->open) {
        h->err = "grape_open_time_gradient: not an open-system handle (grape_create_open); grape_get_time_gradient is the call for a closed one";
        return GRAPE_ERR_INVALID;
    }
    return open_time_gradient(h, dJdt);
}
GRAPE_BARRIER(h ? &h->err : &g_create_error)

int grape_open_hvp(grape_handle *h, int nv, const double *V, double *HV) try {
    if (!h) { g_create_error = "grape_open_hvp: h == NULL"; return GRAPE_ERR_INVALID; }
    if (nv <= 0 || !V || !HV) { h->err = "grape_open_hvp: nv must be positive, V and HV must not be NULL"; return GRAPE_ERR_INVALID; }
    if (!h->open) {
        h->err = "grape_open_hvp: not an open-system handle (grape_create_open); grape_hvp is the call for a closed one";
        return GRAPE_ERR_INVALID;
    }
    return open_hvp(h, nv, V, HV);
}
GRAPE_BARRIER(h ? &h->err : &g_create_error)

// ... 769 lines not shown
```

### grape.jl_amd/csrc/grape_kernels.hip.h

```cpp
#pragma once
#include <hip/hip_runtime.h>
#include <stdint.h>

#include "grape_t18_coeffs.h"

typedef double d4 __attribute__((ext_vector_type(4)));

#define MFMA64(a, b, c) __builtin_amdgcn_mfma_f64_16x16x4f64((a), (b), (c), 0, 0, 0)

__device__ __constant__ double c_pade3[4] = {120., 60., 12., 1.};
__device__ __constant__ double c_pade5[6] = {30240., 15120., 3360., 420., 30., 1.};
__device__ __constant__ double c_pade7[8] = {17297280., 8648640., 1995840., 277200., 25200., 1512., 56., 1.};
__device__ __constant__ double c_pade9[10] = {17643225600., 8821612800., 2075673600., 302702400.,
                                              30270240., 2162160., 110880., 3960., 90., 1.};
#define B13_0 64764752532480000.
#define B13_1 32382376266240000.
#define B13_2 7771770303897600.
#define B13_3 1187353796428800.
#define B13_4 129060195264000.
#define B13_5 10559470521600.
#define B13_6 670442572800.
#define B13_7 33522128640.
#define B13_8 1323241920.
#define B13_9 40840800.
#define B13_10 960960.
#define B13_11 16380.
#define B13_12 182.
#define B13_13 1.

#define GRAPE_STAT_SHARDS 64
#define GRAPE_STAT_SLOTS 16
__device__ __forceinline__ void stat_add(unsigned long long *stats, int idx, unsigned long long v) {
    atomicAdd(&stats[(size_t)(blockIdx.x & (GRAPE_STAT_SHARDS - 1)) * GRAPE_STAT_SLOTS + idx], v);
}

struct ExpmArgs {
    const double *H0f;
    const double *Hcf;
    const double *eps;
    const double *shape;
    const double *dts;
    double2 *U;
    int *flags;
    unsigned long long *stats;
    int K, L, N_T, hc_per_traj;
    const int *rep;
    int *cellflag;
    const double *n1;
    int n1_k;
    int *cell_list;
    int listed;
    const double *Sf;
#ifdef GRAPE_DIAG
    int ablate;
    unsigned long long *stamps;
#endif
};

#define T16_PLAN_R 1.15
#define T16_PLAN_RS 1.11
#define T16_PLAN_SMAX 3
struct T16PlanArgs {
    const double *gram;
    const double *eps, *shape, *dts;
    int *flags;
    int KC, L, N_T, N;
    int *splan;
    int sq_on;
    const double *cert;
    const int *cert_exp;
    int n8, n6;
    int *verdict;
};
#define T16_PLAN_SQ_MASK 0xFF
#define T16_PLAN_CERT 0x100
__device__ __forceinline__ bool t16_certified(const double *t, const int *ex, const int n8, const int n6, const int L, const double *e,
                                              const double dt, const int sq) {
    double p[2] = {0., 0.}, S8 = 0.;
    for (int i = 0; i < n8 + n6; ++i) {
        unsigned x = (unsigned)ex[i];
        double mono = 1.0;
        for (int l = 0; l < L; ++l, x >>= 4)
            for (unsigned q = x & 15u; q > 0; --q) mono *= e[l];
        const double c = t[i];
        p[i < n8 ? 0 : 1] += c * mono;
        if (i < n8) S8 += fabs(c) * fabs(mono);
    }
    const double dt2 = dt * dt, dt8 = (dt2 * dt2) * (dt2 * dt2);
    constexpr double th2 = T16_THETA * T16_THETA, th8 = (th2 * th2) * (th2 * th2);
    const double lhs = (p[0] + 0x1p-30 * S8) * dt8 * (1.0 + 1e-6), rhs = ldexp(th8, 8 * sq);
    return lhs <= rhs && p[1] >= 0.0;
}
__global__ void __launch_bounds__(256) t16_plan_kernel(T16PlanArgs a) {
    const int cell = blockIdx.x * 256 + threadIdx.x;
    bool out = false;
    if (cell < a.KC * a.N_T) {
        const int kc = cell / a.N_T, n = cell - kc * a.N_T, M = a.L + 1;
        const double *G = a.gram + (size_t)kc * (M * M + M), *kap = G + M * M;
        double e[9];
        e[0] = 1.0;
        for (int l = 0; l < a.L; ++l) e[1 + l] = a.eps[(size_t)l * a.N_T + n] * (a.shape ? a.shape[(size_t)l * a.N_T + n] : 1.0);
        double m2 = 0., wk = 0., w = 0.;
        for (int i = 0; i < M; ++i) {
            for (int j = 0; j < M; ++j) m2 += e[i] * e[j] * G[i * M + j];
            const double wi = fabs(e[i]) * sqrt(fmax(G[i * M + i], 0.0));
            w += wi; wk += wi * kap[i];
        }
        const double dt = a.dts[n];
        const double r = 2.0 * fabs(dt) * sqrt(fmax(m2, 0.0) / (double)a.N) * (w > 0.0 ? wk / w : 1.0);
        out = !(r <= T16_PLAN_R);
        if (a.splan) {
            int sq = 0;
            if (out && a.sq_on) {
                double rs = r;
                while (sq < T16_PLAN_SMAX && !(rs <= T16_PLAN_RS)) { rs *= 0.5; ++sq; }
                out = !(rs <= T16_PLAN_RS);
                if (out) sq = 0;
            }
            const bool cert = a.cert && t16_certified(a.cert + (size_t)kc * (a.n8 + a.n6), a.cert_exp, a.n8, a.n6, a.L, e + 1, dt, sq);
            if (cert) a.verdict[cell] = 0;
            a.splan[cell] = sq | (cert ? T16_PLAN_CERT : 0);
        }
    }
    const unsigned long long m = __ballot(out);
    if ((threadIdx.x & 63) == 0 && m) atomicAdd(&a.flags[6], (int)__popcll(m));
}
__device__ __forceinline__ bool t16_skipped(const int *flags, const int ncell) { return 4L * flags[6] > (long)ncell; }

struct CtrlSumArgs {
    const double *Hcf, *eps, *shape;
    double *Sf;
    int L, N_T, pp2;
    int per_traj;
    const int *rep;
};
__device__ __forceinline__ void ctrl_sum_body(CtrlSumArgs a) {
    const int blk = blockIdx.x, kc = a.per_traj ? blk / a.N_T : 0, n = blk - kc * a.N_T;
    if (a.per_traj) a.Hcf += (size_t)(a.rep ? a.rep[kc] : kc) * a.L * a.pp2;
    double e[8];
    for (int l = 0; l < a.L; ++l) e[l] = a.eps[(size_t)l * a.N_T + n] * (a.shape ? a.shape[(size_t)l * a.N_T + n] : 1.0);
    double2 *dst = (double2 *)(a.Sf + (size_t)blk * a.pp2);
#pragma unroll 4
    for (int i = blockIdx.y * blockDim.x + threadIdx.x; i < a.pp2 / 2; i += gridDim.y * blockDim.x) {
        double2 acc = make_double2(0., 0.);
        for (int l = 0; l < a.L; ++l) {
            const double2 h = ((const double2 *)(a.Hcf + (size_t)l * a.pp2))[i];
            acc.x = fma(e[l], h.x, acc.x); acc.y = fma(e[l], h.y, acc.y);
        }
        dst[i] = acc;
    }
}
__global__ void __launch_bounds__(256) ctrl_sum_kernel(CtrlSumArgs a) { ctrl_sum_body(a); }

__global__ void __launch_bounds__(256) dte_kernel(const double *eps, const double *shape, const double *dts, int L, int N_T, int slots, double *out) {
    const int n = blockIdx.x * blockDim.x + threadIdx.x;
    if (n >= N_T) return;
    double *row = out + (size_t)2 * slots * n;
    row[0] = dts[n];
    for (int l = 0; l < 2 * slots - 1; ++l)
        row[1 + l] = l < L ? eps[(size_t)l * N_T + n] * (shape ? shape[(size_t)l * N_T + n] : 1.0) : 0.0;
}

template <int NT>
struct Strip {
    d4 re[NT];
    d4 im[NT];
};

template <int NT>
__device__ __forceinline__ void strip_zero(Strip<NT> &s) {
#pragma unroll
    for (int t = 0; t < NT; ++t) {
        s.re[t] = (d4){0., 0., 0., 0.};
        s.im[t] = (d4){0., 0., 0., 0.};
    }
}

template <int NT>
struct Strip3 {
    d4 p1[NT], p2[NT], p3[NT];
};
template <int NT>
__device__ __forceinline__ void strip3_zero(Strip3<NT> &q) {
#pragma unroll
    for (int t = 0; t < NT; ++t) { q.p1[t] = (d4){0., 0., 0., 0.}; q.p2[t] = (d4){0., 0., 0., 0.}; q.p3[t] = (d4){0., 0., 0., 0.}; }
}
template <int NT>
__device__ __forceinline__ void strip3_add_to(const Strip3<NT> &q, Strip<NT> &acc) {
#pragma unroll
    for (int t = 0; t < NT; ++t) {
        acc.re[t] += q.p1[t] - q.p2[t];
        acc.im[t] += q.p3[t] - q.p1[t] - q.p2[t];
    }
}

template <int NT, int LD>
__device__ __forceinline__ void gemm_xb3(Strip3<NT> &q, const double *__restrict__ Xre,
                                         const double *__restrict__ Xim, const Strip<NT> &B, int lane) {
    const double *__restrict__ xr = Xre + (lane & 15) * LD + (lane >> 4);
    const double *__restrict__ xi = Xim + (lane & 15) * LD + (lane >> 4);
    double are[NT], aim[NT];
#pragma unroll
    for (int tr = 0; tr < NT; ++tr) {
        are[tr] = xr[16 * tr * LD];
// ... 2706 lines not shown
                        const size_t o = (size_t)(16 * rt + 4 * r + rg) * 16 + c;
                        vn[((1 + l) * 2 + 0) * vplane + o] = phr[l][r];
                        vn[((1 + l) * 2 + 1) * vplane + o] = phi[l][r];
                        orr += phr[l][r] * psr[tt][r] + phi[l][r] * psi_[tt][r];
                        oi += phr[l][r] * psi_[tt][r] - phi[l][r] * psr[tt][r];
                        nn += phr[l][r] * phr[l][r] + phi[l][r] * phi[l][r];
                    }
                    orr += __shfl_xor(orr, 16, 64); oi += __shfl_xor(oi, 16, 64); nn += __shfl_xor(nn, 16, 64);
                    orr += __shfl_xor(orr, 32, 64); oi += __shfl_xor(oi, 32, 64); nn += __shfl_xor(nn, 32, 64);
                    sor[l] += orr; soi[l] += oi; snn[l] += nn;
                }
            }
            if (lane < 16) {
#pragma unroll
                for (int l = 0; l < LMAX; ++l) {
                    red[slot][wave][l][c][0] = sor[l];
                    red[slot][wave][l][c][1] = soi[l];
                    red[slot][wave][l][c][2] = snn[l];
                }
            }
            __syncthreads();
            const double al2 = alr * alr + ali * ali;
#pragma unroll
            for (int l = 0; l < LMAX; ++l) {
                if (l < L && !((done_mask >> l) & 1)) {
                    double orr = 0., oi = 0., nn = 0.;
#pragma unroll
                    for (int w = 0; w < NW; ++w) {
                        orr += red[slot][w][l][c][0]; oi += red[slot][w][l][c][1]; nn += red[slot][w][l][c][2];
                    }
                    accr[l] += alr * orr + ali * oi;
                    acci[l] += alr * oi - ali * orr;
                    if (m >= 2 && al2 * nn < a.tol * a.tol) done_mask |= 1 << l;
                }
            }
            cur ^= 1;
            if (__all(done_mask == all_done)) { converged = 1; m_used = m; break; }
            {
                const double f = dt / (double)(m + 1);
                const double nr = -ali * f, ni = alr * f;
                alr = nr; ali = ni;
            }
        }
        if (tid < 16 && valid) {
            for (int l = 0; l < L; ++l) {
                double gr_ = 0., gi_ = 0.;
#pragma unroll
                for (int ll = 0; ll < LMAX; ++ll) if (ll == l) { gr_ = accr[ll]; gi_ = acci[ll]; }
                a.tg[((size_t)k * L + l) * a.N_T + n] = make_double2(rho * gr_, rho * gi_);
            }
        }
        if (tid == 0) {
            const bool redone = a.batch_flag && a.batch_flag[batch];
            if (!converged && !redone) atomicOr(&a.flags[0], 4);
            if (!redone) stat_add(a.stats, 8, (unsigned long long)m_used * (unsigned long long)min(16, a.N_T - n0));
        }
        __syncthreads();
    }
}

struct DerivFlagArgs {
    const double *rb, *eps, *shape, *dts;
    int rb_k, K, L, N_T, hc_per_traj, batches_per_k, nbatch_total;
    double sub_theta;
    int *batch_flag, *flags;
};
__global__ void deriv_flag_kernel(DerivFlagArgs a) {
    const int batch = blockIdx.x * blockDim.x + threadIdx.x;
    if (batch >= a.nbatch_total) return;
    const int k = batch / a.batches_per_k, n0 = (batch - k * a.batches_per_k) * 16;
    int ns = 1;
    for (int n = n0; n < min(n0 + 16, a.N_T); ++n)
        ns = max(ns, deriv_substeps(a.rb, a.rb_k, a.sub_theta, k, a.hc_per_traj, a.L, a.eps, a.shape, a.N_T, n, a.dts[n]));
    a.batch_flag[batch] = ns > 1;
    if (ns > 1) atomicAdd(&a.flags[3], 1);
}

struct DerivEconArgs {
    const int *verdict, *splan, *cls, *flags;
    const int *cell_deg;
    int K, KC, N_T, batches_per_k, nbatch_total;
    int deg0, deg1;
    int *batch_econ;
};
__global__ void deriv_econ_kernel(DerivEconArgs a) {
    const int batch = blockIdx.x * blockDim.x + threadIdx.x;
    if (batch >= a.nbatch_total) return;
    const int k = batch / a.batches_per_k, n0 = (batch - k * a.batches_per_k) * 16;
    const int kc = a.cls ? a.cls[k] : k;
    bool ok = a.cell_deg || !t16_skipped(a.flags, a.KC * a.N_T);
    int deg = 0;
    for (int n = n0; ok && n < min(n0 + 16, a.N_T); ++n) {
        const int cell = kc * a.N_T + n;
        int d;
        if (a.cell_deg) d = a.cell_deg[cell];
        else {
            const int sq = a.splan ? (a.splan[cell] & T16_PLAN_SQ_MASK) : 0;
            d = a.verdict[cell] != 0 ? 0 : sq == 0 ? a.deg0 : sq == 1 ? a.deg1 : 0;
        }
        ok = d > 0;
        deg = max(deg, d);
    }
    a.batch_econ[batch] = ok ? deg : 0;
}

struct DerivSubArgs {
    DerivMfmaArgs m;
    const double *rb;
    int rb_k;
    double sub_theta;
    const int *batch_flag;
};

template <int NP, int LMAX>
__global__ void __launch_bounds__((NP / 16 <= 8 ? NP / 16 : 8) * 64) deriv_sub_kernel(DerivSubArgs b) {
    const DerivMfmaArgs &a = b.m;
    constexpr int RT = NP / 16, KS = NP / 4;
    constexpr int NW = RT <= 8 ? RT : 8, TPW = RT / NW, NV = 1 + LMAX;
    static_assert(RT % NW == 0, "row tiles must divide evenly over the waves");
    __shared__ double red[2][NW][NV][16];
    __shared__ double redo[NW][LMAX][16][2];
    if (b.batch_flag && a.flags[3] == 0) return;
    const int tid = threadIdx.x, lane = tid & 63;
    const int wave = __builtin_amdgcn_readfirstlane(tid >> 6);
    const int c = lane & 15, rg = lane >> 4;
    const int L = a.L;
    const size_t vplane = (size_t)NP * 16;
    double *vbase = a.vecs + (size_t)blockIdx.x * 2 * NV * 2 * vplane;
    for (int batch = blockIdx.x; batch < a.nbatch_total; batch += gridDim.x) {
        if (b.batch_flag && !b.batch_flag[batch]) continue;
        const int k = batch / a.batches_per_k;
        const int n0 = (batch - k * a.batches_per_k) * 16;
        const int n = n0 + c;
        const bool valid = n < a.N_T;
        const int nc = valid ? n : a.N_T - 1;
        const double *h0k = a.H0p + (size_t)k * RT * KS * 128;
        const double *hck = a.Hcp + (size_t)(a.hc_per_traj ? k : 0) * L * RT * KS * 128;
        const double dt = a.dts[nc];
        double e[LMAX], sh[LMAX];
#pragma unroll
        for (int l = 0; l < LMAX; ++l) {
            sh[l] = (l < L && a.shape) ? a.shape[(size_t)l * a.N_T + nc] : 1.0;
            e[l] = l < L ? a.eps[(size_t)l * a.N_T + nc] * sh[l] : 0.;
        }
        int nsub = valid ? deriv_substeps(b.rb, b.rb_k, b.sub_theta, k, a.hc_per_traj, L, a.eps, a.shape, a.N_T, nc, dt) : 1;
#pragma unroll
        for (int off = 1; off < 16; off <<= 1) nsub = max(nsub, __shfl_xor(nsub, off, 64));
        nsub = __builtin_amdgcn_readfirstlane(nsub);
        const double dts_ = dt / (double)nsub;
        const double rho = a.rho[k];
        double psr[TPW][4], psi_[TPW][4];
        d4 chr[TPW], chi_[TPW], gfr[LMAX][TPW], gfi[LMAX][TPW];
#pragma unroll
        for (int tt = 0; tt < TPW; ++tt) {
#pragma unroll
            for (int r = 0; r < 4; ++r) {
                const int row = 16 * (wave + tt * NW) + 4 * r + rg;
                const double2 p = a.fw[((size_t)k * (a.N_T + 1) + nc) * NP + row];
                const double2 x = a.bw[((size_t)k * (a.N_T + 1) + nc + 1) * NP + row];
                psr[tt][r] = p.x; psi_[tt][r] = p.y;
                chr[tt][r] = valid ? x.x : 0.; chi_[tt][r] = valid ? x.y : 0.;
            }
#pragma unroll
            for (int l = 0; l < LMAX; ++l) { gfr[l][tt] = (d4){0., 0., 0., 0.}; gfi[l][tt] = (d4){0., 0., 0., 0.}; }
        }
        const int all_done = ((1 << L) - 1) | (1 << LMAX);
        int converged = 1;
        unsigned long long orders = 0;
        for (int sub = 0; sub < nsub; ++sub) {
            __syncthreads();
#pragma unroll
            for (int tt = 0; tt < TPW; ++tt)
#pragma unroll
                for (int r = 0; r < 4; ++r) {
                    const size_t o = (size_t)(16 * (wave + tt * NW) + 4 * r + rg) * 16 + c;
                    vbase[0 * vplane + o] = chr[tt][r];
                    vbase[1 * vplane + o] = chi_[tt][r];
#pragma unroll
                    for (int l = 0; l < LMAX; ++l) {
                        vbase[((1 + l) * 2 + 0) * vplane + o] = gfr[l][tt][r];
                        vbase[((1 + l) * 2 + 1) * vplane + o] = gfi[l][tt][r];
// ... 301 lines not shown
        int cur = 0, M = 0, converged = 0;
        const int deg = (a.batch_econ && a.batch_flag && a.econ_pairs && !use_g) ? a.batch_flag[a.nbatch_total + batch] : 0;
        const int capb = (deg && deg - 1 <= mcap) ? deg - 1 : mcap;
        const double *pairs = nullptr;
        if (use_g) {
            int mm = Mc;
#pragma unroll
            for (int off = 1; off < 16; off <<= 1) mm = max(mm, __shfl_xor(mm, off, 64));
            M = __builtin_amdgcn_readfirstlane(mm);
            converged = 1;
        } else {
        const double *h0q = a.H0q + (size_t)k * RT * KS * 128, *hcq = a.Hcq + kc;
        load_frags(h0q, hcq);
#pragma unroll
        for (int tt = 0; tt < TPW; ++tt)
#pragma unroll
            for (int r = 0; r < 4; ++r) {
                const int row = 16 * (wave + tt * NW) + 4 * r + rg;
                const double2 p = a.fw[((size_t)k * (a.N_T + 1) + nc) * NP + row];
                const double pr_ = valid ? p.x : 0., pi_ = valid ? p.y : 0.;
                const size_t o = (size_t)row * 16 + c;
                dsm2[o] = pr_; dsm2[vplane + o] = pi_;
                park[o] = pr_; park[vplane + o] = pi_;
            }
        __syncthreads();
        for (int m = 1; m <= capb; ++m) {
            const double *vc = dsm2 + (size_t)cur * 2 * vplane;
            double *vn = dsm2 + (size_t)(ONEBUF ? cur : cur ^ 1) * 2 * vplane;
            const double sfac = dt / (double)m;
            double nn = 0.;
            double keep_r[ONEBUF ? TPW : 1][4], keep_i[ONEBUF ? TPW : 1][4];
#pragma unroll
            for (int tt = 0; tt < TPW; ++tt) {
                const int rt = wave + tt * NW;
                d4 pr[STREAM_L ? 1 : NV], pi[STREAM_L ? 1 : NV];
                if constexpr (STREAM_L) {
                    product1(h0q, vc, rt, pr[0], pi[0]);
                    for (int l = 0; l < L; ++l) {
                        d4 qr, qi;
                        product1(hcq + (size_t)l * RT * KS * 128, vc, rt, qr, qi);
                        pr[0] += e[l] * qr; pi[0] += e[l] * qi;
                    }
                } else {
                    products(h0q, hcq, vc, rt, pr, pi);
#pragma unroll
                    for (int l = 0; l < LMAX; ++l) { pr[0] += e[l] * pr[1 + l]; pi[0] += e[l] * pi[1 + l]; }
                }
#pragma unroll
                for (int r = 0; r < 4; ++r) {
                    const size_t o = (size_t)(16 * rt + 4 * r + rg) * 16 + c;
                    const double ur = sfac * pi[0][r], ui = -sfac * pr[0][r];
                    if constexpr (ONEBUF) { keep_r[ONEBUF ? tt : 0][r] = ur; keep_i[ONEBUF ? tt : 0][r] = ui; }
                    else { vn[o] = ur; vn[vplane + o] = ui; }
#ifdef GRAPE_DIAG
                    if (!(a.ablate & 1))
#endif
                    if (m < a.maxm) { park[(size_t)m * 2 * vplane + o] = ur; park[(size_t)m * 2 * vplane + vplane + o] = ui; }
                    nn += ur * ur + ui * ui;
                }
            }
            if constexpr (ONEBUF) {
                __syncthreads();
#pragma unroll
                for (int tt = 0; tt < TPW; ++tt)
#pragma unroll
                    for (int r = 0; r < 4; ++r) {
                        const size_t o = (size_t)(16 * (wave + tt * NW) + 4 * r + rg) * 16 + c;
                        vn[o] = keep_r[ONEBUF ? tt : 0][r]; vn[vplane + o] = keep_i[ONEBUF ? tt : 0][r];
                    }
            }
            nn += __shfl_xor(nn, 16, 64);
            nn += __shfl_xor(nn, 32, 64);
            if (lane < 16) redn[m & 1][wave][c] = nn;
            __syncthreads();
            double tot = 0.;
#pragma unroll
            for (int w = 0; w < NW; ++w) tot += redn[m & 1][w][c];
            if constexpr (!ONEBUF) cur ^= 1;
            M = m;
            if (m >= 2 && __all(tot < a.tol * a.tol)) { converged = 1; break; }
        }
        if (!converged && capb != mcap) {
            M = deg; converged = 1;
            pairs = a.econ_pairs + (size_t)(deg - 16) * 64;
        }
        }

        const double *h0p = a.H0p + (size_t)k * RT * KS * 128, *hcp = a.Hcp + kc;
        load_frags(h0p, hcp);
        double chr[TPW][4], chi_[TPW][4];
        __syncthreads();
        cur = 0;
#pragma unroll
        for (int tt = 0; tt < TPW; ++tt)
#pragma unroll
            for (int r = 0; r < 4; ++r) {
                const int row = 16 * (wave + tt * NW) + 4 * r + rg;
                const double2 x = a.bw[((size_t)k * (a.N_T + 1) + nc + 1) * NP + row];
                chr[tt][r] = valid ? x.x : 0.; chi_[tt][r] = valid ? x.y : 0.;
                dsm2[(size_t)row * 16 + c] = chr[tt][r];
                dsm2[vplane + (size_t)row * 16 + c] = chi_[tt][r];
            }
        __syncthreads();
        double dr[LMAX], di[LMAX];
#pragma unroll
        for (int l = 0; l < LMAX; ++l) { dr[l] = 0.; di[l] = 0.; }
        for (int aa = M - 1; aa >= 0; --aa) {
            const double *vc = dsm2 + (size_t)cur * 2 * vplane;
            double *vn = dsm2 + (size_t)(ONEBUF ? cur : cur ^ 1) * 2 * vplane;
            const double inv = pairs ? pairs[2 * aa] : 1.0 / (double)(aa + 1), sfac = dt * (pairs ? pairs[2 * aa + 1] : inv);
            double keep_r[ONEBUF ? TPW : 1][4], keep_i[ONEBUF ? TPW : 1][4];
#pragma unroll
            for (int tt = 0; tt < TPW; ++tt) {
                const int rt = wave + tt * NW;
                double ur[4], ui[4];
#pragma unroll
                for (int r = 0; r < 4; ++r) {
                    if (use_g) {
                        const double2 u = a.gpark[(((size_t)k * a.N_T + nc) * a.maxp + aa) * NP + 16 * rt + 4 * r + rg];
                        const bool in = valid && aa < Mc;
                        ur[r] = in ? u.x : 0.; ui[r] = in ? u.y : 0.;
                    } else {
                        const size_t o = (size_t)aa * 2 * vplane + (size_t)(16 * rt + 4 * r + rg) * 16 + c;
#ifdef GRAPE_DIAG
                        if (a.ablate & 1) { ur[r] = chr[tt][r]; ui[r] = chi_[tt][r]; } else
#endif
                        { ur[r] = park[o]; ui[r] = park[vplane + o]; }
                    }
                }
                d4 pr[STREAM_L ? 1 : NV], pi[STREAM_L ? 1 : NV];
                if constexpr (STREAM_L) {
                    product1(h0p, vc, rt, pr[0], pi[0]);
#pragma unroll
                    for (int l = 0; l < LMAX; ++l) {
                        if (l < L) {
                            d4 qr, qi;
                            product1(hcp + (size_t)l * RT * KS * 128, vc, rt, qr, qi);
                            double sr = 0., si = 0.;
#pragma unroll
                            for (int r = 0; r < 4; ++r) {
                                sr += qr[r] * ur[r] + qi[r] * ui[r];
                                si += qr[r] * ui[r] - qi[r] * ur[r];
                            }
                            dr[l] += inv * sr; di[l] += inv * si;
                            pr[0] += e[l] * qr; pi[0] += e[l] * qi;
                        }
                    }
                } else {
                products(h0p, hcp, vc, rt, pr, pi);
#pragma unroll
                for (int l = 0; l < LMAX; ++l) {
                    double sr = 0., si = 0.;
#pragma unroll
                    for (int r = 0; r < 4; ++r) {
                        sr += pr[1 + l][r] * ur[r] + pi[1 + l][r] * ui[r];
                        si += pr[1 + l][r] * ui[r] - pi[1 + l][r] * ur[r];
                    }
                    dr[l] += inv * sr; di[l] += inv * si;
                    pr[0] += e[l] * pr[1 + l]; pi[0] += e[l] * pi[1 + l];
                }
                }
                if (aa > 0) {
#pragma unroll
                    for (int r = 0; r < 4; ++r) {
                        const size_t o = (size_t)(16 * rt + 4 * r + rg) * 16 + c;
                        const double wr_ = chr[tt][r] - sfac * pi[0][r], wi_ = chi_[tt][r] + sfac * pr[0][r];
                        if constexpr (ONEBUF) { keep_r[ONEBUF ? tt : 0][r] = wr_; keep_i[ONEBUF ? tt : 0][r] = wi_; }
// ... 125 lines not shown
```

### grape.jl_amd/csrc/grape_t18.hip

```cpp
#include <hip/hip_runtime.h>
#include <stdint.h>
#include <string.h>
#include <type_traits>
#include <mutex>
#include <vector>
#include <stdlib.h>
#include <stdio.h>
namespace {
#include "grape_t18.hip.h"
#define GRAPE_BATCH_T18_UNIT
#include "grape_batch.hip.h"
#include "grape_deriv3.hip.h"
#include "grape_econ_coeffs.h"

template <int NT, bool SYM, bool CHEB, bool T16 = false>
hipError_t launch(const ExpmArgs &a, hipStream_t s, int blocks) {
    static size_t lds_set[64] = {0};
    const size_t lds = sizeof(double) * (size_t)T18Lds<NT>::TOTAL;
    int dev = 0;
    hipGetDevice(&dev);
    if (lds_set[dev & 63] < lds) {
        hipError_t e = hipFuncSetAttribute((const void *)expm_t18_kernel<NT, SYM, CHEB, T16>, hipFuncAttributeMaxDynamicSharedMemorySize, (int)lds);
        if (e != hipSuccess) return e;
        lds_set[dev & 63] = lds;
// ... 156 lines not shown
    if (cell < ncell) {
        const double bound = expm_norm_bound(a, cell);
        cert = bound > 2.1 && bound <= 5.4;
        if (!cert) todo[atomicAdd(&ntodo, 1)] = cell;
    }
    const unsigned long long m_cert = __ballot(cert);
    if (lane == 0 && m_cert) atomicAdd(&cnt[2 + 4], (unsigned long long)__popcll(m_cert));
    __syncthreads();
    const int nt = ntodo;
    for (int q = 0; q < nt; ++q) {
        const double nA = t16_post_norm1(a, todo[q], red, tid);
        if (tid == 0) {
            const int sj = squarings_of(nA);
            if (sj) { cnt[0] += (unsigned long long)sj; cnt[1] = max(cnt[1], (unsigned long long)sj); }
            cnt[2 + order_of(nA)] += 1ull;
        }
    }
    __syncthreads();
    if (tid == 0) {
        if (cnt[0]) stat_add(a.stats, 0, cnt[0]);
        for (int o = 0; o < 5; ++o)
            if (cnt[2 + o]) stat_add(a.stats, 3 + o, cnt[2 + o]);
        if (cnt[1]) atomicMax(&a.flags[1], (int)cnt[1]);
    }
}

constexpr int D3_INV_TABLE = 2048;
constexpr int D3_PAIRS_OFF = 32768, D3_ECON_OFF = 32768, D3_ECON_TAB_B = 512;
struct AsmModule {
    hipModule_t mod = nullptr;
    hipFunction_t fn = nullptr, fn_d3 = nullptr, fn_d3s = nullptr, fn_lg = nullptr, fn_d3g = nullptr, fn_d4[2] = {nullptr, nullptr};
    hipFunction_t fn_t18g = nullptr, fn_t16p = nullptr, fn_t16p4 = nullptr, fn_t18gp = nullptr;
    double *inv = nullptr;
};
hipError_t asm_function(int dev, hipFunction_t *fn, hipFunction_t *fn_d3 = nullptr, const double **inv = nullptr,
                        hipFunction_t *fn_d3s = nullptr, hipFunction_t *fn_lg = nullptr, hipFunction_t *fn_d3g = nullptr,
                        hipFunction_t *fn_d4 = nullptr, int d4_index = 0, hipFunction_t *fn_t18g = nullptr,
                        hipFunction_t *fn_t16p = nullptr, int t16p_slots = 2) {
    static AsmModule mods[64];
    static std::mutex mtx;
    std::lock_guard<std::mutex> lock(mtx);
    AsmModule &m = mods[dev & 63];
    if (!m.fn) {
        static std::vector<char> override_co;
        const void *image = (const void *)grape_asm_co_start;
        if (const char *path = getenv("GRAPE_ASM_CO")) {
            if (override_co.empty()) {
                if (FILE *f = fopen(path, "rb")) {
                    fseek(f, 0, SEEK_END);
                    const long n = ftell(f);
                    fseek(f, 0, SEEK_SET);
                    if (n > 0) {
                        override_co.resize((size_t)n);
                        if (fread(override_co.data(), 1, (size_t)n, f) != (size_t)n) override_co.clear();
                    }
                    fclose(f);
                }
            }
            if (override_co.empty()) return hipErrorFileNotFound;
            image = override_co.data();
        }
        hipError_t e = hipModuleLoadData(&m.mod, image);
        if (e != hipSuccess) return e;
        e = hipModuleGetFunction(&m.fn_d3, m.mod, "deriv3_asm");
        if (e != hipSuccess) return e;
        e = hipModuleGetFunction(&m.fn_d3s, m.mod, "deriv3s_asm");
        if (e != hipSuccess) return e;
        e = hipModuleGetFunction(&m.fn_lg, m.mod, "lg_gemm_asm");
        if (e != hipSuccess) return e;
        e = hipModuleGetFunction(&m.fn_d3g, m.mod, "deriv3g_asm");
        if (e != hipSuccess) return e;
        e = hipModuleGetFunction(&m.fn_d4[0], m.mod, "deriv4_asm_128");
        if (e != hipSuccess) return e;
        e = hipModuleGetFunction(&m.fn_d4[1], m.mod, "deriv4_asm_256");
        if (e != hipSuccess) return e;
        e = hipModuleGetFunction(&m.fn_t18g, m.mod, "expm_t18g_asm");
        if (e != hipSuccess) return e;
        e = hipModuleGetFunction(&m.fn_t16p, m.mod, "expm_t16p_asm");
        if (e != hipSuccess) return e;
        e = hipModuleGetFunction(&m.fn_t16p4, m.mod, "expm_t16p4_asm");
        if (e != hipSuccess) return e;
        e = hipModuleGetFunction(&m.fn_t18gp, m.mod, "expm_t18gp_asm");
        if (e != hipSuccess) return e;
        static_assert(D3_PAIRS_OFF >= (D3_INV_TABLE + 20) * 8 && D3_ECON_OFF == D3_INV_TABLE * 16 && ECON_MAXDEG <= 31, "layout of gen_d3.py");
        std::vector<double> tab((D3_PAIRS_OFF + D3_ECON_OFF + 16 * D3_ECON_TAB_B) / 8);
        tab[0] = 0.0;
        for (int i = 1; i < D3_INV_TABLE; ++i) tab[i] = 1.0 / (double)i;
        for (int a = 0; a < D3_INV_TABLE; ++a) tab[D3_PAIRS_OFF / 8 + 2 * a] = tab[D3_PAIRS_OFF / 8 + 2 * a + 1] = 1.0 / (double)(a + 1);
        for (int i = 0; i < ECON_NSETS; ++i)
            for (int a = 0; a < ECON_DEG[i]; ++a)
                for (int j = 0; j < 2; ++j)
                    tab[(D3_PAIRS_OFF + D3_ECON_OFF + (ECON_DEG[i] - 16) * D3_ECON_TAB_B) / 8 + 2 * a + j] = ECON_TABS[i][a][j];
        int *pt = (int *)(tab.data() + D3_INV_TABLE);
        int np_ = 0;
        for (int ti = 0; ti < 4; ++ti)
            for (int tj = ti; tj < 4; ++tj)
                for (int plane = 0; plane < 2; ++plane)
                    for (int half = 0; half < 2; ++half) pt[np_++] = plane * 64 * 64 * 8 + ti * 16 * 64 * 8 + tj * 16 * 8;
        e = hipMalloc((void **)&m.inv, sizeof(double) * tab.size());
        if (e != hipSuccess) return e;
        e = hipMemcpy(m.inv, tab.data(), sizeof(double) * tab.size(), hipMemcpyHostToDevice);
        if (e != hipSuccess) return e;
        e = hipModuleGetFunction(&m.fn, m.mod, "expm_t16_asm");
        if (e != hipSuccess) return e;
    }
    if (fn) *fn = m.fn;
    if (fn_d3) *fn_d3 = m.fn_d3;
    if (fn_d3s) *fn_d3s = m.fn_d3s;
    if (fn_lg) *fn_lg = m.fn_lg;
    if (fn_d3g) *fn_d3g = m.fn_d3g;
    if (fn_d4) *fn_d4 = m.fn_d4[d4_index & 1];
    if (fn_t18g) *fn_t18g = m.fn_t18g;
    if (fn_t16p) *fn_t16p = t16p_slots == 4 ? m.fn_t16p4 : t16p_slots == 0 ? m.fn_t18gp : m.fn_t16p;
    if (inv) *inv = m.inv;
    return hipSuccess;
}
}

namespace {
struct D3AsmArgs {
    const double *H0f, *Hcf, *eps, *shape, *dts;
    const double2 *fw, *bw;
    const double *rho;
    double2 *tg;
    double *park;
    int *flags;
    unsigned long long *stats;
    const int *batch_flag;
    const double *inv;
    int K, L, N_T, hc_per_traj, wpt, batches_per_k, mcap, slots;
    double tol2;
    int deep, nblocks;
};
static_assert(sizeof(D3AsmArgs) == 160, "argument block of the assembly kernel");

hipError_t launch_d3_asm(const Deriv3Args &g, hipStream_t s, int blocks, bool general) {
    const Deriv2Args &a = g.d;
    if (a.L < 1 || a.L > (general ? 7 : 8) || blocks < 1 || a.maxm + 2 > D3_INV_TABLE) return hipErrorInvalidValue;
    if ((long)a.N_T + 1 >= (1L << 21) || (long)a.K * a.L * a.N_T >= (1L << 27)) return hipErrorInvalidValue;
    int dev = 0;
    hipError_t e = hipGetDevice(&dev);
    if (e != hipSuccess) return e;
    hipFunction_t fn, fn_s, fn_g;
    const double *inv;
    e = asm_function(dev, nullptr, &fn, &inv, &fn_s, nullptr, &fn_g);
    if (e != hipSuccess) return e;
    if (a.L > 2) fn = fn_s;
    if (general) fn = fn_g;
    D3AsmArgs k{};
    k.H0f = g.H0f; k.Hcf = g.Hcf; k.eps = a.eps; k.shape = a.shape; k.dts = a.dts; k.fw = a.fw; k.bw = a.bw; k.rho = a.rho;
    k.tg = a.tg; k.park = a.park; k.flags = a.flags; k.stats = a.stats; k.batch_flag = a.batch_flag; k.inv = inv;
    k.K = a.K; k.L = a.L; k.N_T = a.N_T; k.hc_per_traj = a.hc_per_traj; k.wpt = g.wpt; k.batches_per_k = a.batches_per_k;
    k.mcap = a.max_order < a.maxm ? a.max_order : a.maxm;
    k.slots = a.maxm + 1;
    k.tol2 = a.tol * a.tol;
    k.deep = (a.deep_redo && a.max_order > k.mcap) ? 1 : 0;
    if (a.batch_econ && !general && a.batch_flag && k.mcap >= ECON_MAXDEG) k.deep |= 2;
    k.nblocks = blocks;
    size_t size = sizeof(k);
    void *cfg[] = {HIP_LAUNCH_PARAM_BUFFER_POINTER, &k, HIP_LAUNCH_PARAM_BUFFER_SIZE, &size, HIP_LAUNCH_PARAM_END};
    return hipModuleLaunchKernel(fn, (unsigned)blocks, 1, 1, 256, 1, 1, 0, s, nullptr, cfg);
}
}

extern "C" const double *grape_econ_pairs(void) {
    int dev = 0;
    if (hipGetDevice(&dev) != hipSuccess) return nullptr;
    hipFunction_t fn;
    const double *inv = nullptr;
    if (asm_function(dev, nullptr, &fn, &inv) != hipSuccess || !inv) return nullptr;
    static_assert(D3_ECON_TAB_B == 64 * 8, "64 doubles per degree");
    return inv + (D3_PAIRS_OFF + D3_ECON_OFF) / 8;
}

namespace {
// ... 241 lines not shown
```

### include/grape_hip.h

```cpp
#ifndef GRAPE_HIP_H
#define GRAPE_HIP_H

#include <stddef.h>
#include <stdint.h>

#ifdef __cplusplus
extern "C" {
#endif

#define GRAPE_HIP_ABI_VERSION 7

typedef struct grape_handle grape_handle;

typedef enum {
    GRAPE_OK = 0,
    GRAPE_ERR_INVALID = -1,
    GRAPE_ERR_HIP = -2,
    GRAPE_ERR_CHI_NORM = -3,
    GRAPE_ERR_SINGULAR = -4,
    GRAPE_ERR_TAYLOR = -5,
    GRAPE_ERR_NO_CONTROLS = -6,
    GRAPE_ERR_AGAIN = -7,
    GRAPE_ERR_HOST = -8
} grape_status;
// ... 8 lines not shown
    GRAPE_GRAD_GRADGEN = 0,
    GRAPE_GRAD_TAYLOR = 1
} grape_gradient_method;

typedef enum {
    GRAPE_PROP_EXP = 0,
    GRAPE_PROP_SERIES = 1
} grape_prop_method;

typedef struct {
    int32_t abi_version;
    int32_t N;
    int32_t L;
    int32_t K;
    int32_t K_total;
    int32_t N_T;
    int32_t functional;
    int32_t gradient_method;
    int32_t hc_per_traj;
    int32_t device;
    const double *tlist;
    const double *H0;
    const double *Hc;
    const double *shape;
    const double *psi0;
    const double *target;
    const double *weights;
    double chi_min_norm;
    int32_t taylor_max_order;
    double taylor_tolerance;
    const double *Dpen;
    int32_t dpen_per_traj;
    double lambda_b;
    int32_t prop_method;
    double prop_tolerance;
    int32_t ndev;
    const int32_t *devices;
    int32_t taylor_no_check;
} grape_problem;

int grape_create(grape_handle **out, const grape_problem *problem);
void grape_destroy(grape_handle *h);

typedef struct {
    int32_t J;
    int32_t cops_per_traj;
    const double *cops;
} grape_lindblad;
int grape_create_open(grape_handle **out, const grape_problem *problem, const grape_lindblad *diss);

int grape_eval(grape_handle *h, const double *pulsevals, double *J, double *G, double *tau,
               double *psiT);

int grape_forward(grape_handle *h, const double *pulsevals, double *tau );
int grape_backward(grape_handle *h, const double f_total[2], double *G_partial);

int grape_get_sums(grape_handle *h, double sums[8]);

int grape_get_final_states(grape_handle *h, double *psiT);

int grape_backward_chi(grape_handle *h, const double *chi, double *G);

int grape_backward_xi(grape_handle *h, const double f_total[2], const double *chi, const double *xi, double lambda_b,
                      double *G);

int grape_forward_device(grape_handle *h, const double *d_pulsevals, double *d_out, void *stream);
int grape_backward_device(grape_handle *h, const double *d_f, double *d_G, void *stream);

int grape_set_fused_sweeps(grape_handle *h, int on);

int grape_check(grape_handle *h, void *stream);

int grape_get_propagator(grape_handle *h, int k, int n, double *out);

int grape_get_tau_grads(grape_handle *h, double *out );
int grape_get_storage(grape_handle *h, int which , double *out );

int grape_get_timings(grape_handle *h, double *ms, int n);
int grape_reset_timings(grape_handle *h);
int grape_get_work(grape_handle *h, double *out, int n);

int grape_get_cert_table(grape_handle *h, int *dims, double *coef, int *exps);

int grape_get_time_gradient(grape_handle *h, double *dJdt );

int grape_open_time_gradient(grape_handle *h, double *dJdt );

int grape_set_tlist(grape_handle *h, const double *tlist );

int grape_eval_batch(grape_handle *h, int P, const double *pulsevals, double *J, double *G, double *tau);

int grape_get_batch_info(grape_handle *h, double *out, int n);

int grape_hvp(grape_handle *h, int nv, const double *V, double *HV);

int grape_get_hvp_info(grape_handle *h, double *out, int n);

int grape_hvp_forward(grape_handle *h, int nv, const double *V, double *dtau, double *dsums, double *dpsiT);
int grape_hvp_backward(grape_handle *h, int nv, const double f_total[2], const double *df_total, double *HV);
int grape_hvp_backward_chi(grape_handle *h, int nv, const double *chi, const double *dchi, double *HV);

int grape_open_hvp(grape_handle *h, int nv, const double *V, double *HV);

int grape_get_open_hvp_info(grape_handle *h, double *out, int n);

int grape_open_hvp_forward(grape_handle *h, int nv, const double *V, double *dtau, double *dsums, double *drhoT);
int grape_open_hvp_backward(grape_handle *h, int nv, const double f_total[2], const double *df_total, double *HV);
int grape_open_hvp_backward_chi(grape_handle *h, int nv, const double *chi, const double *dchi, double *HV);

int grape_open_eval_batch(grape_handle *h, int P, const double *pulsevals, double *J, double *G, double *tau);

int grape_get_open_batch_info(grape_handle *h, double *out, int n);

int grape_open_set_running_cost(grape_handle *h, const double *D, int d_per_traj, double lambda_b);

int grape_open_backward_xi(grape_handle *h, const double f_total[2], const double *chi, const double *xi, double lambda_b,
                           double *G);

const char *grape_last_error(grape_handle *h);
int grape_abi_version(void);

#ifdef __cplusplus
}
#endif
#endif
```

Baseline: 54.50.

## Add certified degree-15 economized derivative series for segments with small spectral bound

Adds a degree-15 economized coefficient set with a smaller theta, and precomputes per-class trace polynomials of degree 4, 8 and 12 moment bounds. A restructured plan kernel, which now caches the tables and control powers in LDS and is templated on L, certifies per cell whether the norm bound fits the smaller theta. When it does, the derivative kernel uses the lower degree, cutting one series term per certified cell. This adds setup cost and plan-kernel work, and only applies for L<=2 with econ derivatives enabled.

```diff
diff --git a/grape.jl_amd/api.py b/grape.jl_amd/api.py
--- a/grape.jl_amd/api.py
+++ b/grape.jl_amd/api.py
@@ -22,7 +22,7 @@
 
 EXPORTS = ["grape_create", "grape_destroy", "grape_eval", "grape_forward", "grape_backward",
            "grape_forward_device", "grape_backward_device", "grape_check", "grape_get_propagator",
-           "grape_get_tau_grads", "grape_get_storage", "grape_get_timings", "grape_reset_timings", "grape_get_work", "grape_get_cert_table",
+           "grape_get_tau_grads", "grape_get_storage", "grape_get_timings", "grape_reset_timings", "grape_get_work", "grape_get_cert_table", "grape_get_seg_table",
            "grape_last_error", "grape_abi_version", "grape_set_fused_sweeps", "grape_get_sums", "grape_backward_xi",
            "grape_get_final_states", "grape_backward_chi",
            "grape_get_time_gradient", "grape_set_tlist", "grape_eval_batch", "grape_get_batch_info", "grape_create_open",
@@ -94,7 +94,7 @@
 def _sources():
     srcs = [os.path.join(_CSRC, f) for f in ("grape_hip.hip", "grape_t18.hip", "grape_kernels.hip.h", "grape_large.hip.h",
                                              "grape_series.hip.h", "grape_cheby.hip.h", "grape_t18.hip.h", "grape_t18_coeffs.h",
-                                             "grape_deriv3.hip.h", "grape_timegrad.hip.h", "grape_batch.hip.h", "grape_lindblad.hip.h", "grape_lindblad_tg.hip.h", "grape_hvp.hip.h", "grape_hvp_split.hip.h", "grape_lindblad_hvp.hip.h", "grape_lindblad_hvp_split.hip.h", "grape_lindblad_batch.hip.h", "grape_lindblad_rc.hip.h", "grape_devmem.h", "grape_cert.hip.h", os.path.join("asm", "gen_t16.py"), os.path.join("asm", "gen_t16p.py"), os.path.join("asm", "gen_t18g.py"), os.path.join("asm", "gen_t18gp.py"), os.path.join("asm", "gen_d3.py"), os.path.join("asm", "gen_d3s.py"), os.path.join("asm", "gen_lg.py"), os.path.join("asm", "gen_d4.py"), os.path.join("asm", "gcn.py"))]
+                                             "grape_deriv3.hip.h", "grape_timegrad.hip.h", "grape_batch.hip.h", "grape_lindblad.hip.h", "grape_lindblad_tg.hip.h", "grape_hvp.hip.h", "grape_hvp_split.hip.h", "grape_lindblad_hvp.hip.h", "grape_lindblad_hvp_split.hip.h", "grape_lindblad_batch.hip.h", "grape_lindblad_rc.hip.h", "grape_devmem.h", "grape_cert.hip.h", "grape_econ_coeffs.h", os.path.join("asm", "gen_t16.py"), os.path.join("asm", "gen_t16p.py"), os.path.join("asm", "gen_t18g.py"), os.path.join("asm", "gen_t18gp.py"), os.path.join("asm", "gen_d3.py"), os.path.join("asm", "gen_d3s.py"), os.path.join("asm", "gen_lg.py"), os.path.join("asm", "gen_d4.py"), os.path.join("asm", "gcn.py"))]
     return srcs, os.path.join(_HERE, "..", "include", "grape_hip.h")
 
 
@@ -181,6 +181,7 @@
     lib.grape_get_timings.argtypes = [vp, vp, ip]
     lib.grape_get_work.argtypes = [vp, vp, ip]
     lib.grape_get_cert_table.argtypes = [vp, vp, vp, vp]
+    lib.grape_get_seg_table.argtypes = [vp, vp, vp, vp]
     lib.grape_reset_timings.argtypes = [vp]
     lib.grape_set_fused_sweeps.argtypes = [vp, ip]
     lib.grape_get_sums.argtypes = [vp, vp]
@@ -494,13 +495,13 @@
         self._chk(self._lib.grape_reset_timings(self._h))
 
     def work(self):
-        w = np.zeros(20)
-        self._lib.grape_get_work(self._h, w.ctypes.data, 20)
+        w = np.zeros(21)
+        self._lib.grape_get_work(self._h, w.ctypes.data, 21)
         return dict(cells=w[0], squarings=w[1], flop_expm=w[2], flop_deriv=w[3], deriv_orders=w[4],
                     pivoted_cells=w[5], expm_cells=w[6], series_terms=w[7], series_steps=w[8],
                     t18_mfma_flop=w[9], t18_squarings=w[10], t18_cells=w[11], matrix_free_fallback=w[12], t16_cells=w[13],
                     asm_kernel=w[14], asm_deriv_kernel=w[15], asm_blocked_products=w[16],
-                    walk_steps=w[17], scan_block=w[18], t16_certified=w[19])
+                    walk_steps=w[17], scan_block=w[18], t16_certified=w[19], seg_certified=w[20])
 
     def cert_table(self):
         dims = np.zeros(3, np.int32)
@@ -511,6 +512,17 @@
             self._chk(self._lib.grape_get_cert_table(self._h, dims.ctypes.data, coef.ctypes.data, exps.ctypes.data))
         ex = np.stack([(exps >> (4 * l)) & 15 for l in range(self.L)], axis=1) if n8 + n6 else np.zeros((0, self.L), np.int32)
         return coef[:, :n8], coef[:, n8:], ex
+
+    def seg_table(self):
+        dims = np.zeros(4, np.int32)
+        self._chk(self._lib.grape_get_seg_table(self._h, dims.ctypes.data, None, None))
+        KC, n4, n8, n12 = (int(x) for x in dims)
+        nt = n4 + n8 + n12
+        coef, exps = np.zeros((KC, nt)), np.zeros(nt, np.int32)
+        if nt:
+            self._chk(self._lib.grape_get_seg_table(self._h, dims.ctypes.data, coef.ctypes.data, exps.ctypes.data))
+        ex = np.stack([(exps >> (4 * l)) & 15 for l in range(self.L)], axis=1) if nt else np.zeros((0, self.L), np.int32)
+        return coef[:, :n4], coef[:, n4:n4 + n8], coef[:, n4 + n8:], ex
 
 
 def liouvillian(H, cops=()):
diff --git a/grape.jl_amd/csrc/asm/gen_d3.py b/grape.jl_amd/csrc/asm/gen_d3.py
--- a/grape.jl_amd/csrc/asm/gen_d3.py
+++ b/grape.jl_amd/csrc/asm/gen_d3.py
@@ -13,7 +13,14 @@
 MAT_B = NTILE * 2 * TILE_B
 KERNARG = 160
 VPLANE_B = NP * 16 * 16
-ECON_MIN = 16
+
+def _econ_mindeg():
+    import re
+    with open(os.path.join(os.path.dirname(os.path.abspath(__file__)), "..", "grape_econ_coeffs.h")) as f:
+        return int(re.search(r"#define ECON_MINDEG (\d+)", f.read()).group(1))
+
+
+ECON_MIN = _econ_mindeg()
 PAIRS_OFF = 32768
 ECON_OFF = 32768
 ECON_TAB_B = 512
diff --git a/grape.jl_amd/csrc/grape_cert.hip.h b/grape.jl_amd/csrc/grape_cert.hip.h
--- a/grape.jl_amd/csrc/grape_cert.hip.h
+++ b/grape.jl_amd/csrc/grape_cert.hip.h
@@ -37,17 +37,17 @@
 };
 
 struct CertPlan {
-    int M, n2, n3, n4, n6, n8, nmat;
-    CertJobs mm2, mm34, tr;
+    int M, n2, n3, n4, n6, n8, n12, nmat;
+    CertJobs mm2, mm34, mm6, tr;
     std::vector<int> exps;
-    explicit CertPlan(int L) {
+    explicit CertPlan(int L, bool seg = false) {
         M = L + 1;
-        const CertMonomials m2(M, 2), m3(M, 3), m4(M, 4), m6(M, 6), m8(M, 8);
-        n2 = m2.size(); n3 = m3.size(); n4 = m4.size(); n6 = m6.size(); n8 = m8.size();
-        const int o2 = M, o3 = o2 + n2, o4 = o3 + n3;
-        nmat = o4 + n4;
+        const CertMonomials m2(M, 2), m3(M, 3), m4(M, 4), m6(M, 6), m8(M, 8), m12(M, 12);
+        n2 = m2.size(); n3 = m3.size(); n4 = m4.size(); n6 = m6.size(); n8 = m8.size(); n12 = seg ? m12.size() : 0;
+        const int o2 = M, o3 = o2 + n2, o4 = o3 + n3, o6 = o4 + n4;
+        nmat = o6 + (seg ? n6 : 0);
         auto var = [&](int a) { return (uint32_t)1 << (4 * a); };
-        std::vector<std::vector<int>> l2(n2), l34(n3 + n4), lt(n8 + n6);
+        std::vector<std::vector<int>> l2(n2), l34(n3 + n4), l6(seg ? n6 : 0), lt(n8 + n6 + (seg ? n4 + n12 : 0));
         for (int a = 0; a < M; ++a)
             for (int b = 0; b < M; ++b) { auto &l = l2[m2.index.at(var(a) + var(b))]; l.push_back(a); l.push_back(b); }
         for (int i = 0; i < n2; ++i)
@@ -58,9 +58,21 @@
             for (int j = 0; j < n4; ++j) { auto &l = lt[m8.index.at(m4.key[i] + m4.key[j])]; l.push_back(o4 + i); l.push_back(o4 + j); }
         for (int i = 0; i < n3; ++i)
             for (int j = 0; j < n3; ++j) { auto &l = lt[n8 + m6.index.at(m3.key[i] + m3.key[j])]; l.push_back(o3 + i); l.push_back(o3 + j); }
-        mm2.from(l2); mm34.from(l34); tr.from(lt);
+        if (seg) {
+            for (int i = 0; i < n3; ++i)
+                for (int j = 0; j < n3; ++j) { auto &l = l6[m6.index.at(m3.key[i] + m3.key[j])]; l.push_back(o3 + i); l.push_back(o3 + j); }
+            for (int i = 0; i < n2; ++i)
+                for (int j = 0; j < n2; ++j) { auto &l = lt[n8 + n6 + m4.index.at(m2.key[i] + m2.key[j])]; l.push_back(o2 + i); l.push_back(o2 + j); }
+            for (int i = 0; i < n6; ++i)
+                for (int j = 0; j < n6; ++j) { auto &l = lt[n8 + n6 + n4 + m12.index.at(m6.key[i] + m6.key[j])]; l.push_back(o6 + i); l.push_back(o6 + j); }
+        }
+        mm2.from(l2); mm34.from(l34); mm6.from(l6); tr.from(lt);
         for (int i = 0; i < n8; ++i) exps.push_back((int)(m8.key[i] >> 4));
         for (int i = 0; i < n6; ++i) exps.push_back((int)(m6.key[i] >> 4));
+        if (seg) {
+            for (int i = 0; i < n4; ++i) exps.push_back((int)(m4.key[i] >> 4));
+            for (int i = 0; i < n12; ++i) exps.push_back((int)(m12.key[i] >> 4));
+        }
     }
 };
 
diff --git a/grape.jl_amd/csrc/grape_deriv3.hip.h b/grape.jl_amd/csrc/grape_deriv3.hip.h
--- a/grape.jl_amd/csrc/grape_deriv3.hip.h
+++ b/grape.jl_amd/csrc/grape_deriv3.hip.h
@@ -196,7 +196,7 @@
             }
             if (!converged && capb != mcap) {
                 M = deg; converged = 1;
-                pairs = a.econ_pairs + (size_t)(deg - 16) * 64;
+                pairs = a.econ_pairs + (size_t)(deg - ECON_MINDEG) * 64;
             }
             Strip<NT> chi;
 #pragma unroll
diff --git a/grape.jl_amd/csrc/grape_econ_coeffs.h b/grape.jl_amd/csrc/grape_econ_coeffs.h
--- a/grape.jl_amd/csrc/grape_econ_coeffs.h
+++ b/grape.jl_amd/csrc/grape_econ_coeffs.h
@@ -1,9 +1,29 @@
 #pragma once
-#define ECON_NSETS 4
+#define ECON_NSETS 5
+#define ECON_MINDEG 15
 #define ECON_MAXDEG 21
-static const int ECON_DEG[4] = {16, 17, 19, 21};
-static const double ECON_THETAS[4] = {1.36, 1.6, 2.0, 2.72};
-static const double ECON_TABS[4][21][2] = {
+#define ECON_SEG_THETA 1.11
+#define ECON_VERDICT_SET 1
+static const int ECON_DEG[5] = {15, 16, 17, 19, 21};
+static const double ECON_THETAS[5] = {1.11, 1.36, 1.6, 2.0, 2.72};
+static const double ECON_TABS[5][21][2] = {
+    {
+        {0.99999999999999999239, 0.0},
+        {0.49999999999999851797, 0.49999999999999852178},
+        {0.3333333333333328058, 0.33333333333333379382},
+        {0.2499999999998652315, 0.24999999999986562716},
+        {0.19999999999993523983, 0.20000000000004305463},
+        {0.16666666665090805766, 0.16666666665096202447},
+        {0.14285714284812829142, 0.14285714286163567056},
+        {0.1249999980801762681, 0.124999998088064013},
+        {0.11111110985838383123, 0.11111111156489382211},
+        {0.099999780383310034409, 0.099999781510762122935},
+        {0.090908931033978596621, 0.090909130685602284833},
+        {0.083311907089360955007, 0.083312053604124151368},
+        {0.076905921260223919788, 0.076925700006016818603},
+        {0.069873048178623135011, 0.069888634994793089618},
+        {0.06531076511119096165, 0.066764722198373690759},
+    },
     {
         {0.99999999999999980529, 0.0},
         {0.49999999999999995125, 0.5000000000000000486},
diff --git a/grape.jl_amd/csrc/grape_hip.hip b/grape.jl_amd/csrc/grape_hip.hip
--- a/grape.jl_amd/csrc/grape_hip.hip
+++ b/grape.jl_amd/csrc/grape_hip.hip
@@ -112,6 +112,11 @@
     double *d_cert = nullptr;
     int *d_cert_exp = nullptr;
     int cert_n8 = 0, cert_n6 = 0;
+    double *d_seg = nullptr;
+    double *d_seg8 = nullptr;
+    int *d_seg_exp = nullptr;
+    int seg_n8 = 0, seg_n4 = 0, seg_n12 = 0, seg8_stride = 0, seg_exp_off = 0;
+    int *d_segplan = nullptr;
     bool asm16 = false;
     bool asm16p = false;
     double *d_dte = nullptr;
@@ -2892,19 +2897,34 @@
         });
         CCHK(h->mem.alloc(&h->d_gram, gram.size()));
         CCHK(hipMemcpy(h->d_gram, gram.data(), gram.size() * 8, hipMemcpyHostToDevice));
-        const char *envc = getenv("GRAPE_EXPM_CERT");
-        if (h->asm16 && L >= 1 && L <= GRAPE_CERT_LMAX && !(envc && atoi(envc) == 0)) {
-            const CertPlan pl(L);
-            const int nt = pl.n8 + pl.n6;
-            h->cert_n8 = pl.n8; h->cert_n6 = pl.n6;
-            CCHK(h->mem.alloc(&h->d_cert, (size_t)KCn * nt));
-            CCHK(h->mem.alloc(&h->d_cert_exp, (size_t)nt));
-            CCHK(hipMemcpy(h->d_cert_exp, pl.exps.data(), (size_t)nt * sizeof(int), hipMemcpyHostToDevice));
+        const char *envc = getenv("GRAPE_EXPM_CERT"), *envg = getenv("GRAPE_DERIV_SEG");
+        static_assert(T16_PLAN_LMAX == GRAPE_CERT_LMAX, "power table of t16_plan_kernel");
+        const bool want_cert = h->asm16 && L >= 1 && L <= GRAPE_CERT_LMAX && !(envc && atoi(envc) == 0);
+        const bool want_seg = h->asm16 && h->deriv_econ && L >= 1 && L <= 2 && !(envg && atoi(envg) == 0);
+        if (want_cert || want_seg) {
+            const CertPlan pl(L, want_seg);
+            const int nt = pl.n8 + pl.n6, ns = pl.n4 + pl.n12;
+            if (want_cert) {
+                h->cert_n8 = pl.n8; h->cert_n6 = pl.n6;
+                CCHK(h->mem.alloc(&h->d_cert, (size_t)KCn * nt));
+                CCHK(h->mem.alloc(&h->d_cert_exp, (size_t)nt));
+                CCHK(hipMemcpy(h->d_cert_exp, pl.exps.data(), (size_t)nt * sizeof(int), hipMemcpyHostToDevice));
+            }
+            if (want_seg) {
+                h->seg_n8 = pl.n8; h->seg_n4 = pl.n4; h->seg_n12 = pl.n12; h->seg_exp_off = nt;
+                CCHK(h->mem.alloc(&h->d_seg, (size_t)KCn * ns));
+                CCHK(h->mem.alloc(&h->d_seg_exp, pl.exps.size()));
+                CCHK(hipMemcpy(h->d_seg_exp, pl.exps.data(), pl.exps.size() * sizeof(int), hipMemcpyHostToDevice));
+                if (want_cert) { h->d_seg8 = h->d_cert; h->seg8_stride = nt; }
+                else { CCHK(h->mem.alloc(&h->d_seg8, (size_t)KCn * pl.n8)); h->seg8_stride = pl.n8; }
+                CCHK(h->mem.alloc(&h->d_segplan, (size_t)KCn * N_T));
+                CCHK(hipMemset(h->d_segplan, 0, (size_t)KCn * N_T * sizeof(int)));
+            }
             DeviceBufs tmp;
-            int *d_job[6] = {nullptr, nullptr, nullptr, nullptr, nullptr, nullptr};
-            const std::vector<int> *job[6] = {&pl.mm2.row, &pl.mm2.pair, &pl.mm34.row, &pl.mm34.pair, &pl.tr.row, &pl.tr.pair};
-            for (int i = 0; i < 6; ++i) {
-                CCHK(tmp.alloc(&d_job[i], job[i]->size()));
+            int *d_job[8] = {nullptr, nullptr, nullptr, nullptr, nullptr, nullptr, nullptr, nullptr};
+            const std::vector<int> *job[8] = {&pl.mm2.row, &pl.mm2.pair, &pl.mm34.row, &pl.mm34.pair, &pl.tr.row, &pl.tr.pair, &pl.mm6.row, &pl.mm6.pair};
+            for (int i = 0; i < 8; ++i) {
+                CCHK(tmp.alloc(&d_job[i], std::max<size_t>(1, job[i]->size())));
                 CCHK(hipMemcpy(d_job[i], job[i]->data(), job[i]->size() * sizeof(int), hipMemcpyHostToDevice));
             }
             const size_t per_class = (size_t)pl.nmat * N * N;
@@ -2918,8 +2938,18 @@
                 hipLaunchKernelGGL(cert_mm_kernel, dim3((unsigned)pl.n2, nc), dim3(256), 0, 0, d_scr, pl.nmat, N, pl.M, (const int *)d_job[0], (const int *)d_job[1]);
                 hipLaunchKernelGGL(cert_mm_kernel, dim3((unsigned)(pl.n3 + pl.n4), nc), dim3(256), 0, 0, d_scr, pl.nmat, N, pl.M + pl.n2, (const int *)d_job[2],
                                    (const int *)d_job[3]);
-                hipLaunchKernelGGL(cert_trace_kernel, dim3((unsigned)nt, nc), dim3(256), 0, 0, (const double2 *)d_scr, pl.nmat, N, (const int *)d_job[4],
-                                   (const int *)d_job[5], nt, h->d_cert + (size_t)kc0 * nt);
+                if (want_cert)
+                    hipLaunchKernelGGL(cert_trace_kernel, dim3((unsigned)nt, nc), dim3(256), 0, 0, (const double2 *)d_scr, pl.nmat, N, (const int *)d_job[4],
+                                       (const int *)d_job[5], nt, h->d_cert + (size_t)kc0 * nt);
+                else
+                    hipLaunchKernelGGL(cert_trace_kernel, dim3((unsigned)pl.n8, nc), dim3(256), 0, 0, (const double2 *)d_scr, pl.nmat, N, (const int *)d_job[4],
+                                       (const int *)d_job[5], pl.n8, h->d_seg8 + (size_t)kc0 * pl.n8);
+                if (want_seg) {
+                    hipLaunchKernelGGL(cert_mm_kernel, dim3((unsigned)pl.n6, nc), dim3(256), 0, 0, d_scr, pl.nmat, N, pl.M + pl.n2 + pl.n3 + pl.n4,
+                                       (const int *)d_job[6], (const int *)d_job[7]);
+                    hipLaunchKernelGGL(cert_trace_kernel, dim3((unsigned)ns, nc), dim3(256), 0, 0, (const double2 *)d_scr, pl.nmat, N,
+                                       (const int *)d_job[4] + nt, (const int *)d_job[5], ns, h->d_seg + (size_t)kc0 * ns);
+                }
                 CCHK(hipGetLastError());
             }
             CCHK(hipDeviceSynchronize());
@@ -3053,7 +3083,18 @@
                     pa.sq_on = h->asm_sq ? 1 : 0;
                     pa.cert = h->d_cert; pa.cert_exp = h->d_cert_exp; pa.n8 = h->cert_n8; pa.n6 = h->cert_n6;
                     pa.verdict = h->d_cellflag;
-                    hipLaunchKernelGGL(t16_plan_kernel, dim3((unsigned)((ncell + 255) / 256)), dim3(256), 0, s, pa);
+                    pa.seg = h->d_seg; pa.seg8 = h->d_seg8; pa.seg8_stride = h->seg8_stride; pa.seg8_exp = h->d_seg_exp;
+                    pa.seg_exp = h->d_seg_exp ? h->d_seg_exp + h->seg_exp_off : nullptr;
+                    pa.s8 = h->seg_n8; pa.n4 = h->seg_n4; pa.n12 = h->seg_n12; pa.segplan = h->d_segplan;
+                    const unsigned plan_blocks = (unsigned)(h->KC * ((h->N_T + T16_PLAN_TPB - 1) / T16_PLAN_TPB));
+                    const size_t plan_lds = t16_plan_lds(pa);
+                    switch (plan_lds ? h->L : 0) {
+                        case 1: hipLaunchKernelGGL(t16_plan_kernel<1>, dim3(plan_blocks), dim3(T16_PLAN_TPB), plan_lds, s, pa); break;
+                        case 2: hipLaunchKernelGGL(t16_plan_kernel<2>, dim3(plan_blocks), dim3(T16_PLAN_TPB), plan_lds, s, pa); break;
+                        case 3: hipLaunchKernelGGL(t16_plan_kernel<3>, dim3(plan_blocks), dim3(T16_PLAN_TPB), plan_lds, s, pa); break;
+                        case 4: hipLaunchKernelGGL(t16_plan_kernel<4>, dim3(plan_blocks), dim3(T16_PLAN_TPB), plan_lds, s, pa); break;
+                        default: hipLaunchKernelGGL(t16_plan_kernel<0>, dim3(plan_blocks), dim3(T16_PLAN_TPB), 0, s, pa); break;
+                    }
                     HIPCHK(h, hipGetLastError());
                 }
                 const int blocks16 = (t16 && h->NT == 3) ? 8 * (int)std::max<long>(1, std::min<long>((long)(h->num_cus / 8) * 2, (ncell + 7) / 8)) : t18_blocks;
@@ -3111,8 +3152,9 @@
             DerivEconArgs ec{};
             ec.verdict = h->d_cellflag; ec.splan = h->d_splan; ec.cls = h->d_cls; ec.flags = h->d_flags;
             ec.cell_deg = h->large ? h->d_celldeg : nullptr;
-            ec.deg0 = ECON_DEG[0]; ec.deg1 = ECON_DEG[ECON_NSETS - 1];
-            static_assert(ECON_NSETS == 4, "segments 1.36 (verdict), 1.6, 2.0 (blocked path), 2.72 (one planned squaring)");
+            ec.deg0 = ECON_DEG[ECON_VERDICT_SET]; ec.deg1 = ECON_DEG[ECON_NSETS - 1];
+            ec.segplan = h->large ? nullptr : h->d_segplan; ec.deg_seg = ECON_DEG[0];
+            static_assert(ECON_NSETS == 5, "segments 1.11 (three-moment certificate), 1.36 (verdict), 1.6, 2.0 (blocked path), 2.72 (one planned squaring)");
             ec.K = h->K; ec.KC = h->KC; ec.N_T = h->N_T; ec.batches_per_k = (h->N_T + 15) / 16;
             ec.nbatch_total = h->K * ec.batches_per_k; ec.batch_econ = h->d_batchflag + ec.nbatch_total;
             hipLaunchKernelGGL(deriv_econ_kernel, dim3((unsigned)((ec.nbatch_total + 255) / 256)), dim3(256), 0, s, ec);
@@ -4129,10 +4171,10 @@
     if (!h || !out || n < 4) return GRAPE_ERR_INVALID;
     if (h->open) return open_work(h, out, n);
     if (!h->shards.empty()) {
-        const int m = n < 20 ? n : 20;
+        const int m = n < 21 ? n : 21;
         std::fill(out, out + m, 0.0);
         for (grape_handle *c : h->shards) {
-            double cw[20] = {0.};
+            double cw[21] = {0.};
             const int rc = grape_get_work(c, cw, m);
             if (rc < 0) return multi_fail(h, c, rc);
             for (int i = 0; i < m; ++i) out[i] = (i == 15 || i == 16 || i == 18) ? cw[i] : out[i] + cw[i];
@@ -4198,17 +4240,30 @@
     }
     if (n > 18) out[18] = h->scan16 ? (double)h->scan_Bk : 0.0;
     if (n > 19) {
-        double certified = 0.0;
-        if (h->d_cert && h->d_splan && !h->series) {
+        double certified = 0.0, seg = 0.0;
+        const bool want_seg = n > 20 && h->d_segplan && h->deriv_econ;
+        if ((h->d_cert || want_seg) && h->d_splan && !h->series) {
             const size_t ncell = (size_t)h->KC * h->N_T;
             std::vector<int> plan(ncell);
             int fl[8];
             HIPCHK(h, hipMemcpy(plan.data(), h->d_splan, ncell * sizeof(int), hipMemcpyDeviceToHost));
             HIPCHK(h, hipMemcpy(fl, h->d_flags, sizeof(fl), hipMemcpyDeviceToHost));
-            if (!(4L * fl[6] > (long)ncell))
+            const bool tried = !(4L * fl[6] > (long)ncell);
+            if (tried && h->d_cert)
                 for (int w : plan) certified += (w & T16_PLAN_CERT) ? 1.0 : 0.0;
+            if (tried && want_seg) {
+                std::vector<int> sp(ncell), verdict(ncell);
+                HIPCHK(h, hipMemcpy(sp.data(), h->d_segplan, ncell * sizeof(int), hipMemcpyDeviceToHost));
+                HIPCHK(h, hipMemcpy(verdict.data(), h->d_cellflag, ncell * sizeof(int), hipMemcpyDeviceToHost));
+                for (int k = 0; k < h->K; ++k) {
+                    const size_t c0 = (size_t)(h->cls.empty() ? k : h->cls[k]) * h->N_T;
+                    for (int i = 0; i < h->N_T; ++i)
+                        seg += (sp[c0 + i] && verdict[c0 + i] == 0 && (plan[c0 + i] & T16_PLAN_SQ_MASK) == 0) ? 1.0 : 0.0;
+                }
+            }
         }
         out[19] = certified;
+        if (n > 20) out[20] = seg;
     }
     return 4;
 }
@@ -4226,6 +4281,33 @@
     HIPCHK(h, hipSetDevice(h->device));
     if (coef) HIPCHK(h, hipMemcpy(coef, h->d_cert, (size_t)h->KC * nt * sizeof(double), hipMemcpyDeviceToHost));
     if (exps) HIPCHK(h, hipMemcpy(exps, h->d_cert_exp, (size_t)nt * sizeof(int), hipMemcpyDeviceToHost));
+    return GRAPE_OK;
+}
+GRAPE_BARRIER(h ? &h->err : &g_create_error)
+
+int grape_get_seg_table(grape_handle *h, int *dims, double *coef, int *exps) try {
+    if (!h || !dims) return GRAPE_ERR_INVALID;
+    if (h->open || !h->shards.empty()) {
+        h->err = "grape_get_seg_table: a closed handle on one device";
+        return GRAPE_ERR_INVALID;
+    }
+    const int n4 = h->seg_n4, n8 = h->seg_n8, n12 = h->seg_n12, nt = n4 + n8 + n12;
+    dims[0] = h->KC; dims[1] = n4; dims[2] = n8; dims[3] = n12;
+    if (!h->d_seg || !nt) { dims[1] = dims[2] = dims[3] = 0; return GRAPE_OK; }
+    HIPCHK(h, hipSetDevice(h->device));
+    if (coef) {
+        HIPCHK(h, hipMemcpy2D(coef, (size_t)nt * sizeof(double), h->d_seg, (size_t)(n4 + n12) * sizeof(double), (size_t)n4 * sizeof(double),
+                              (size_t)h->KC, hipMemcpyDeviceToHost));
+        HIPCHK(h, hipMemcpy2D(coef + n4, (size_t)nt * sizeof(double), h->d_seg8, (size_t)h->seg8_stride * sizeof(double), (size_t)n8 * sizeof(double),
+                              (size_t)h->KC, hipMemcpyDeviceToHost));
+        HIPCHK(h, hipMemcpy2D(coef + n4 + n8, (size_t)nt * sizeof(double), h->d_seg + n4, (size_t)(n4 + n12) * sizeof(double), (size_t)n12 * sizeof(double),
+                              (size_t)h->KC, hipMemcpyDeviceToHost));
+    }
+    if (exps) {
+        HIPCHK(h, hipMemcpy(exps, h->d_seg_exp + h->seg_exp_off, (size_t)n4 * sizeof(int), hipMemcpyDeviceToHost));
+        HIPCHK(h, hipMemcpy(exps + n4, h->d_seg_exp, (size_t)n8 * sizeof(int), hipMemcpyDeviceToHost));
+        HIPCHK(h, hipMemcpy(exps + n4 + n8, h->d_seg_exp + h->seg_exp_off + n4, (size_t)n12 * sizeof(int), hipMemcpyDeviceToHost));
+    }
     return GRAPE_OK;
 }
 GRAPE_BARRIER(h ? &h->err : &g_create_error)
diff --git a/grape.jl_amd/csrc/grape_kernels.hip.h b/grape.jl_amd/csrc/grape_kernels.hip.h
--- a/grape.jl_amd/csrc/grape_kernels.hip.h
+++ b/grape.jl_amd/csrc/grape_kernels.hip.h
@@ -3,6 +3,7 @@
 #include <stdint.h>
 
 #include "grape_t18_coeffs.h"
+#include "grape_econ_coeffs.h"
 
 typedef double d4 __attribute__((ext_vector_type(4)));
 
@@ -71,31 +72,96 @@
     const int *cert_exp;
     int n8, n6;
     int *verdict;
+    const double *seg;
+    const double *seg8;
+    const int *seg_exp;
+    const int *seg8_exp;
+    int seg8_stride, s8, n4, n12;
+    int *segplan;
 };
 #define T16_PLAN_SQ_MASK 0xFF
 #define T16_PLAN_CERT 0x100
-__device__ __forceinline__ bool t16_certified(const double *t, const int *ex, const int n8, const int n6, const int L, const double *e,
-                                              const double dt, const int sq) {
-    double p[2] = {0., 0.}, S8 = 0.;
-    for (int i = 0; i < n8 + n6; ++i) {
-        unsigned x = (unsigned)ex[i];
-        double mono = 1.0;
-        for (int l = 0; l < L; ++l, x >>= 4)
-            for (unsigned q = x & 15u; q > 0; --q) mono *= e[l];
-        const double c = t[i];
-        p[i < n8 ? 0 : 1] += c * mono;
-        if (i < n8) S8 += fabs(c) * fabs(mono);
-    }
+#define T16_PLAN_TPB 128
+#define T16_PLAN_LMAX 4
+#define T16_PLAN_PMAX 12
+typedef double T16PlanPowers[T16_PLAN_PMAX + 1][T16_PLAN_TPB];
+template <int LT>
+__device__ __forceinline__ void t16_trace_poly(const double *t, const int *ex, const int n, const T16PlanPowers *pw, double &p, double &S) {
+    const int tid = threadIdx.x;
+    double sp = 0., sa = 0.;
+    for (int i0 = 0; i0 < n; i0 += 8) {
+        unsigned x[8];
+        double c[8], mono[8];
+#pragma unroll
+        for (int u = 0; u < 8; ++u) {
+            const int i = min(i0 + u, n - 1);
+            x[u] = (unsigned)ex[i];
+            c[u] = i0 + u < n ? t[i] : 0.0;
+        }
+#pragma unroll
+        for (int u = 0; u < 8; ++u) {
+            mono[u] = pw[0][x[u] & 15u][tid];
+#pragma unroll
+            for (int l = 1; l < LT; ++l) mono[u] *= pw[l][(x[u] >> (4 * l)) & 15u][tid];
+        }
+#pragma unroll
+        for (int u = 0; u < 8; ++u) {
+            sp += c[u] * mono[u];
+            sa += fabs(c[u]) * fabs(mono[u]);
+        }
+    }
+    p = sp; S = sa;
+}
+__device__ __forceinline__ bool t16_certified(const double p8, const double S8, const double p6, const double dt, const int sq) {
     const double dt2 = dt * dt, dt8 = (dt2 * dt2) * (dt2 * dt2);
     constexpr double th2 = T16_THETA * T16_THETA, th8 = (th2 * th2) * (th2 * th2);
-    const double lhs = (p[0] + 0x1p-30 * S8) * dt8 * (1.0 + 1e-6), rhs = ldexp(th8, 8 * sq);
-    return lhs <= rhs && p[1] >= 0.0;
-}
-__global__ void __launch_bounds__(256) t16_plan_kernel(T16PlanArgs a) {
-    const int cell = blockIdx.x * 256 + threadIdx.x;
+    const double lhs = (p8 + 0x1p-30 * S8) * dt8 * (1.0 + 1e-6), rhs = ldexp(th8, 8 * sq);
+    return lhs <= rhs && p6 >= 0.0;
+}
+__device__ __forceinline__ bool t16_seg_certified(const double p4, const double S4, const double p8, const double S8, const double p12,
+                                                  const double S12, const double dt) {
+    constexpr double th = ECON_SEG_THETA, th2 = th * th, th4 = th2 * th2, th8 = th4 * th4, th12 = th8 * th4;
+    const double dt2 = dt * dt, dt4 = dt2 * dt2, dt8 = dt4 * dt4, dt12 = dt8 * dt4;
+    const double m4lo = (p4 - 0x1p-30 * S4) * dt4, m4hi = (p4 + 0x1p-30 * S4) * dt4;
+    const double m8lo = (p8 - 0x1p-30 * S8) * dt8, m8hi = (p8 + 0x1p-30 * S8) * dt8;
+    const double m12hi = (p12 + 0x1p-30 * S12) * dt12;
+    if (m4hi * (1.0 + 1e-6) <= th4) return true;
+    if (!(m8hi * (1.0 + 1e-6) < th4 * m4lo)) return false;
+    const double lo = m8lo - th8, hi = m8hi - th8;
+    const double gap = lo > 0.0 ? lo : hi < 0.0 ? -hi : 0.0;
+    const double lhs = (m12hi - th12) * (m4hi - th4);
+    return (lhs > 0.0 ? lhs * (1.0 + 1e-6) : lhs) < gap * gap;
+}
+struct T16PlanLds {
+    int nc, n8own, ns;
+    __host__ __device__ explicit T16PlanLds(const T16PlanArgs &a)
+        : nc(a.cert ? a.n8 + a.n6 : 0), n8own((a.seg && !a.cert) ? a.s8 : 0), ns(a.seg ? a.n4 + a.n12 : 0) {}
+    __host__ __device__ int entries() const { return nc + n8own + ns; }
+};
+__host__ __device__ inline size_t t16_plan_lds(const T16PlanArgs &a) {
+    if (!(a.cert || a.seg) || a.L > T16_PLAN_LMAX) return 0;
+    return (size_t)a.L * sizeof(T16PlanPowers) + (size_t)T16PlanLds(a).entries() * (sizeof(double) + sizeof(int));
+}
+template <int LT>
+__global__ void __launch_bounds__(T16_PLAN_TPB) t16_plan_kernel(T16PlanArgs a) {
+    extern __shared__ __attribute__((aligned(16))) double plan_sm[];
+    const int tid = threadIdx.x, nbx = (a.N_T + T16_PLAN_TPB - 1) / T16_PLAN_TPB;
+    const int kc = blockIdx.x / nbx, n = (blockIdx.x - kc * nbx) * T16_PLAN_TPB + tid;
+    constexpr bool tables = LT > 0;
+    T16PlanPowers *pw = (T16PlanPowers *)plan_sm;
+    const T16PlanLds ly(a);
+    const int nc = ly.nc, n8own = ly.n8own, ns = ly.ns;
+    double *tt = plan_sm + (size_t)LT * (T16_PLAN_PMAX + 1) * T16_PLAN_TPB;
+    int *tx = (int *)(tt + ly.entries());
+    if (tables) {
+        for (int i = tid; i < nc; i += T16_PLAN_TPB) { tt[i] = a.cert[(size_t)kc * nc + i]; tx[i] = a.cert_exp[i]; }
+        for (int i = tid; i < n8own; i += T16_PLAN_TPB) { tt[nc + i] = a.seg8[(size_t)kc * a.seg8_stride + i]; tx[nc + i] = a.seg8_exp[i]; }
+        for (int i = tid; i < ns; i += T16_PLAN_TPB) { tt[nc + n8own + i] = a.seg[(size_t)kc * ns + i]; tx[nc + n8own + i] = a.seg_exp[i]; }
+        __syncthreads();
+    }
     bool out = false;
-    if (cell < a.KC * a.N_T) {
-        const int kc = cell / a.N_T, n = cell - kc * a.N_T, M = a.L + 1;
+    if (n < a.N_T) {
+        const int cell = kc * a.N_T + n, M = a.L + 1;
         const double *G = a.gram + (size_t)kc * (M * M + M), *kap = G + M * M;
         double e[9];
         e[0] = 1.0;
@@ -109,17 +175,43 @@
         const double dt = a.dts[n];
         const double r = 2.0 * fabs(dt) * sqrt(fmax(m2, 0.0) / (double)a.N) * (w > 0.0 ? wk / w : 1.0);
         out = !(r <= T16_PLAN_R);
+        int sq = 0;
+        if (a.splan && out && a.sq_on) {
+            double rs = r;
+            while (sq < T16_PLAN_SMAX && !(rs <= T16_PLAN_RS)) { rs *= 0.5; ++sq; }
+            out = !(rs <= T16_PLAN_RS);
+            if (out) sq = 0;
+        }
+        if (tables)
+            for (int l = 0; l < LT; ++l) {
+                double x = 1.0;
+                for (int j = 0; j <= T16_PLAN_PMAX; ++j, x *= e[1 + l]) pw[l][j][tid] = x;
+            }
+        double p8 = 0., S8 = 0.;
+        const bool have8 = a.splan && a.cert;
         if (a.splan) {
-            int sq = 0;
-            if (out && a.sq_on) {
-                double rs = r;
-                while (sq < T16_PLAN_SMAX && !(rs <= T16_PLAN_RS)) { rs *= 0.5; ++sq; }
-                out = !(rs <= T16_PLAN_RS);
-                if (out) sq = 0;
-            }
-            const bool cert = a.cert && t16_certified(a.cert + (size_t)kc * (a.n8 + a.n6), a.cert_exp, a.n8, a.n6, a.L, e + 1, dt, sq);
+            bool cert = false;
+            if (tables && a.cert) {
+                double p6, S6;
+                t16_trace_poly<LT>(tt, tx, a.n8, pw, p8, S8);
+                t16_trace_poly<LT>(tt + a.n8, tx + a.n8, a.n6, pw, p6, S6);
+                cert = t16_certified(p8, S8, p6, dt, sq);
+            }
             if (cert) a.verdict[cell] = 0;
             a.splan[cell] = sq | (cert ? T16_PLAN_CERT : 0);
+        }
+        if (tables && a.seg) {
+            bool seg = false;
+            if (sq == 0) {
+                const double *t = tt + nc + n8own;
+                const int *x = tx + nc + n8own;
+                double p4, S4, p12, S12;
+                if (!have8) t16_trace_poly<LT>(a.cert ? tt : tt + nc, a.cert ? tx : tx + nc, a.s8, pw, p8, S8);
+                t16_trace_poly<LT>(t, x, a.n4, pw, p4, S4);
+                t16_trace_poly<LT>(t + a.n4, x + a.n4, a.n12, pw, p12, S12);
+                seg = t16_seg_certified(p4, S4, p8, S8, p12, S12, dt);
+            }
+            a.segplan[cell] = seg ? 1 : 0;
         }
     }
     const unsigned long long m = __ballot(out);
@@ -2992,6 +3084,8 @@
     int K, KC, N_T, batches_per_k, nbatch_total;
     int deg0, deg1;
     int *batch_econ;
+    const int *segplan;
+    int deg_seg;
 };
 __global__ void deriv_econ_kernel(DerivEconArgs a) {
     const int batch = blockIdx.x * blockDim.x + threadIdx.x;
@@ -3007,6 +3101,7 @@
         else {
             const int sq = a.splan ? (a.splan[cell] & T16_PLAN_SQ_MASK) : 0;
             d = a.verdict[cell] != 0 ? 0 : sq == 0 ? a.deg0 : sq == 1 ? a.deg1 : 0;
+            if (d == a.deg0 && sq == 0 && a.segplan && a.segplan[cell]) d = a.deg_seg;
         }
         ok = d > 0;
         deg = max(deg, d);
@@ -3474,7 +3569,7 @@
         }
         if (!converged && capb != mcap) {
             M = deg; converged = 1;
-            pairs = a.econ_pairs + (size_t)(deg - 16) * 64;
+            pairs = a.econ_pairs + (size_t)(deg - ECON_MINDEG) * 64;
         }
         }
 
diff --git a/grape.jl_amd/csrc/grape_t18.hip b/grape.jl_amd/csrc/grape_t18.hip
--- a/grape.jl_amd/csrc/grape_t18.hip
+++ b/grape.jl_amd/csrc/grape_t18.hip
@@ -262,7 +262,7 @@
         if (e != hipSuccess) return e;
         e = hipModuleGetFunction(&m.fn_t18gp, m.mod, "expm_t18gp_asm");
         if (e != hipSuccess) return e;
-        static_assert(D3_PAIRS_OFF >= (D3_INV_TABLE + 20) * 8 && D3_ECON_OFF == D3_INV_TABLE * 16 && ECON_MAXDEG <= 31, "layout of gen_d3.py");
+        static_assert(D3_PAIRS_OFF >= (D3_INV_TABLE + 20) * 8 && D3_ECON_OFF == D3_INV_TABLE * 16 && ECON_MAXDEG - ECON_MINDEG <= 15, "layout of gen_d3.py");
         std::vector<double> tab((D3_PAIRS_OFF + D3_ECON_OFF + 16 * D3_ECON_TAB_B) / 8);
         tab[0] = 0.0;
         for (int i = 1; i < D3_INV_TABLE; ++i) tab[i] = 1.0 / (double)i;
@@ -270,7 +270,7 @@
         for (int i = 0; i < ECON_NSETS; ++i)
             for (int a = 0; a < ECON_DEG[i]; ++a)
                 for (int j = 0; j < 2; ++j)
-                    tab[(D3_PAIRS_OFF + D3_ECON_OFF + (ECON_DEG[i] - 16) * D3_ECON_TAB_B) / 8 + 2 * a + j] = ECON_TABS[i][a][j];
+                    tab[(D3_PAIRS_OFF + D3_ECON_OFF + (ECON_DEG[i] - ECON_MINDEG) * D3_ECON_TAB_B) / 8 + 2 * a + j] = ECON_TABS[i][a][j];
         int *pt = (int *)(tab.data() + D3_INV_TABLE);
         int np_ = 0;
         for (int ti = 0; ti < 4; ++ti)
diff --git a/include/grape_hip.h b/include/grape_hip.h
--- a/include/grape_hip.h
+++ b/include/grape_hip.h
@@ -114,6 +114,8 @@
 
 int grape_get_cert_table(grape_handle *h, int *dims, double *coef, int *exps);
 
+int grape_get_seg_table(grape_handle *h, int *dims, double *coef, int *exps);
+
 int grape_get_time_gradient(grape_handle *h, double *dJdt );
 
 int grape_open_time_gradient(grape_handle *h, double *dJdt );
```

Result: faster. 55.28 (median of 6 runs) (+1.4%).
